# ZephirFXEC/HNanoSolver

Measured on AMD Instinct MI355X. Metric: solver substeps/sec (advect + 50 red-black SOR iterations + project) at N active voxels, higher is better.
Workload: dtype f32

## Files before the change

### hnanosolver_amd/_lib.py

```python
from __future__ import annotations

import ctypes as C
import os

_HERE = os.path.dirname(os.path.abspath(__file__))
_LIB_PATH = os.environ.get("HNS_LIBRARY") or os.path.join(_HERE, "lib", "libhns.so")

HNS_OK = 0
HNS_ERR_INVALID_ARGUMENT = -1
HNS_ERR_RUNTIME = -2
HNS_ERR_HIP = -3
HNS_ERR_NO_DEVICE = -4
HNS_ERR_TOPOLOGY = -5

HNS_GRID_DEFAULT = 0
HNS_GRID_HOST_ONLY = 1
HNS_GRID_SKIP_VALIDATE = 2


class HNSError(RuntimeError):

    def __init__(self, code: int, message: str):
        super().__init__(f"libhns error {code}: {message}")
        self.code = code
        self.message = message


class hns_field(C.Structure):
    _fields_ = [("name", C.c_char_p), ("ncomp", C.c_int), ("host", C.POINTER(C.c_float))]


class hns_dist_stats(C.Structure):
    _fields_ = [("world", C.c_int), ("rank", C.c_int), ("peers", C.c_int), ("sweeps_per_exchange", C.c_int),
                ("boundary_leaves", C.c_uint64), ("interior_leaves", C.c_uint64), ("ghost_leaves", C.c_uint64),
                ("region_voxels_sent", C.c_uint64 * 4), ("bytes_sent", C.c_uint64 * 4), ("messages_sent", C.c_uint64), ("exchanges", C.c_uint64),
                ("halo_peers", C.c_uint64), ("packed_exchanges", C.c_uint64), ("chained", C.c_uint64)]


HNS_DIST_IPC_BLOB_BYTES = 2048
HNS_DIST_PLAN_ONLY = 1
HNS_DIST_LEAF_ORDER = 2


class hns_leaf_source(C.Structure):
    _fields_ = [("name", C.c_char_p), ("ncomp", C.c_int), ("origins", C.c_void_p), ("n_leaves", C.c_uint64), ("masks", C.c_void_p), ("values", C.c_void_p)]


class hns_activity_field(C.Structure):
    _fields_ = [("name", C.c_char_p), ("ncomp", C.c_int), ("tolerance", C.c_float)]


class hns_combustion_params(C.Structure):
    _fields_ = [(n, C.c_float) for n in ("expansionRate", "temperatureRelease", "buoyancyStrength", "ambientTemp", "vorticityScale", "factorScale")]


_vp, _i, _u64, _f = C.c_void_p, C.c_int, C.c_uint64, C.c_float
_fp = C.c_void_p
_ip = C.POINTER(C.c_int)

SIGNATURES = {
    "hns_last_error": (C.c_char_p, []),
    "hns_version": (_i, []),
    "hns_device_count": (_i, []),
    "hns_trim_memory": (_i, []),
    "hns_set_option": (_i, [C.c_char_p, C.c_char_p]),
    "hns_get_option": (C.c_char_p, [C.c_char_p]),
    "hns_grid_create": (_vp, [_vp, _u64, _f, C.c_uint, _ip]),
    "hns_grid_create_from_leaves": (_vp, [_vp, _u64, _f, C.c_uint, _ip]),
    "hns_grid_destroy": (None, [_vp]),
    "hns_grid_leaf_count": (_u64, [_vp]),
    "hns_grid_voxel_count": (_u64, [_vp]),
    "hns_grid_voxel_size": (_f, [_vp]),
    "hns_grid_set_active_leaves": (_i, [_vp, _u64]),
    "hns_grid_set_active_range": (_i, [_vp, _u64, _u64]),
    "hns_grid_active_leaves": (_u64, [_vp]),
    "hns_grid_set_outside_element": (_i, [_vp, _u64]),
    "hns_grid_offsets": (_i, [_vp, _vp, _u64, _vp]),
    "hns_grid_neighbor_table": (_i, [_vp, _vp]),
    "hns_grid_coords": (_i, [_vp, _vp]),
    "hns_grid_release_cache": (_i, [_vp]),
    "hns_grid_matches": (_i, [_vp, _vp, _u64, C.c_uint]),
    "hns_grid_export_nanovdb": (_i, [_vp, _vp, _u64, _vp]),
    "hns_grid_launch_tables": (_i, [_vp, _vp]),
    "hns_gather_leaves": (_i, [_vp, _u64, _vp, _u64, _vp, _i, _i, _vp]),
    "hns_scatter_leaves": (_i, [_vp, _u64, _i, C.POINTER(C.c_void_p)]),
    "hns_dilate_leaves": (_i, [_vp, _u64, _vp, _i, _vp, _u64, C.POINTER(C.c_uint64)]),
    "hns_dilate_leaf_masks": (_i, [_vp, _u64, _vp, _i, _vp, _vp, _u64, C.POINTER(C.c_uint64)]),
    "hns_union_leaves": (_i, [_vp, _u64, _vp, _u64, _vp, _u64, C.POINTER(C.c_uint64)]),
    "hns_add_leaves": (_i, [_vp, _u64, _vp, _vp, _vp, _u64, _vp, _vp, _i, _vp, _vp, _vp, _u64, C.POINTER(C.c_uint64)]),
    "hns_deactivate_leaf_masks": (_i, [_u64, _vp, C.POINTER(hns_activity_field), C.POINTER(C.c_void_p), _i, _vp, C.POINTER(C.c_uint64)]),
    "hns_compute_sim": (_i, [_vp, C.POINTER(hns_field), _i, _i, _f, _f, C.POINTER(hns_combustion_params), _i, _vp]),
    "hns_compute_sim_resident": (_i, [_vp, C.POINTER(hns_field), _i, C.c_char_p, C.POINTER(C.c_int), _i, _f, _f, C.POINTER(hns_combustion_params), _i, _vp]),
    "hns_advect_index_grid": (_i, [_vp, C.POINTER(hns_field), _i, _f, _f, _vp]),
    "hns_advect_index_grid_velocity": (_i, [_vp, C.POINTER(hns_field), _i, _f, _f, _vp]),
    "hns_project_non_divergent": (_i, [_vp, C.POINTER(hns_field), _i, _u64, _f, _vp]),
    "hns_divergence": (_i, [_vp, C.POINTER(hns_field), _i, _f, _vp]),
    "hns_sim_create": (_vp, [_vp, C.POINTER(C.c_char_p), _i, _ip]),
    "hns_sim_destroy": (None, [_vp]),
    "hns_sim_upload": (_i, [_vp, C.POINTER(hns_field), _i, _vp]),
    "hns_sim_download": (_i, [_vp, C.POINTER(hns_field), _i, _vp]),
    "hns_sim_substep": (_i, [_vp, _i, _f, _f, C.POINTER(hns_combustion_params), _i, _vp]),
    "hns_sim_core_substep": (_i, [_vp, _i, _f, _f, _vp]),
    "hns_sim_pressure_solve": (_i, [_vp, _i, _f, _vp]),
    "hns_sim_timing": (_i, [_vp, _i]),
    "hns_sim_pressure_time": (_i, [_vp, C.POINTER(C.c_float), C.POINTER(C.c_longlong)]),
    "hns_sim_stage_timing": (_i, [_vp, _i]),
    "hns_sim_stage_times": (_i, [_vp, C.POINTER(C.c_float), C.POINTER(C.c_longlong)]),
    "hns_sim_velocity_ptr": (_vp, [_vp]),
    "hns_sim_field_ptr": (_vp, [_vp, C.c_char_p]),
    "hns_sim_divergence_ptr": (_vp, [_vp]),
    "hns_sim_pressure_ptr": (_vp, [_vp]),
    "hns_sim_set_active_masks": (_i, [_vp, _vp, _vp]),
    "hns_sim_active_masks": (_i, [_vp, _vp, _vp]),
    "hns_sim_regrid": (_vp, [_vp, _i, _vp, _u64, _vp, _vp, _vp, _ip]),
    "hns_sim_regrid_times": (_i, [_vp, C.POINTER(C.c_float)]),
    "hns_sim_regrid_sourced": (_vp, [_vp, _i, C.POINTER(hns_leaf_source), _i, _vp, _u64, _vp, _vp, _vp, _ip]),
    "hns_sim_deactivate": (_i, [_vp, C.POINTER(hns_activity_field), _i, C.POINTER(C.c_uint64), _vp]),
    "hns_dev_advect_vector": (_i, [_vp, _fp, _fp, _fp, _i, _f, _f, _vp]),
    "hns_dev_advect_scalar": (_i, [_vp, _fp, _fp, _fp, _fp, _i, _f, _f, _vp]),
    "hns_dev_advect_scalars": (_i, [_vp, _fp, C.POINTER(C.c_void_p), C.POINTER(C.c_void_p), _i, _fp, _i, _f, _f, _vp]),
    "hns_dev_divergence": (_i, [_vp, _fp, _fp, _f, _vp]),
    "hns_dev_rbgs_color": (_i, [_vp, _fp, _fp, _f, _f, _i, _vp]),
    "hns_dev_rbgs_iterate": (_i, [_vp, _fp, _fp, _fp, _f, _f, _i, _ip, _vp]),
    "hns_dev_subtract_pressure_gradient": (_i, [_vp, _fp, _fp, _fp, _fp, _i, _f, _vp]),
    "hns_dev_combustion_oxygen": (_i, [_fp] * 9 + [_f, _f, _u64, _vp]),
    "hns_dev_temperature_buoyancy": (_i, [_fp, _fp, _fp, _f, _f, _f, _u64, _vp]),
    "hns_dev_vorticity_confinement": (_i, [_vp, _fp, _fp, _f, _f, _f, _f, _vp]),
    "hns_dev_enforce_collision_boundaries": (_i, [_vp, _fp, _fp, _f, _vp]),
    "hns_dev_pack_leaves": (_i, [_fp, _vp, _u64, _fp, _i, _vp]),
    "hns_dev_unpack_leaves": (_i, [_fp, _vp, _u64, _fp, _i, _vp]),
    "hns_dist_create": (_vp, [_vp, _u64, _i, _i, _f, _i, _i, C.c_uint, _ip]),
    "hns_dist_destroy": (None, [_vp]),
    "hns_dist_unique_id": (_i, [_vp]),
    "hns_dist_connect_rccl": (_i, [_vp, _vp]),
    "hns_dist_connect_local": (_i, [C.POINTER(C.c_void_p), _i]),
    "hns_dist_connect_loopback": (_i, [_vp]),
    "hns_dist_connect_loopback_rccl": (_i, [_vp]),
    "hns_dist_ipc_export": (_i, [_vp, _vp]),
    "hns_dist_connect_ipc": (_i, [_vp, _vp]),
    "hns_dist_owned_leaves": (_u64, [_vp]),
    "hns_dist_first_owned_leaf": (_u64, [_vp]),
    "hns_dist_owned_leaf_ids": (_i, [_vp, _vp]),
    "hns_dist_partition_axis": (_i, [_vp]),
    "hns_dist_one_sided_sweeps": (_i, [_u64, _i]),
    "hns_dist_info": (_i, [_vp, C.POINTER(hns_dist_stats)]),
    "hns_dist_local_leaves": (_i, [_vp, _vp]),
    "hns_dist_peer_rank": (_i, [_vp, _i]),
    "hns_dist_peer_region": (_i, [_vp, _i, _i, _i, _vp, _vp, C.POINTER(C.c_uint64), C.POINTER(C.c_uint64)]),
    "hns_dist_upload": (_i, [_vp, _vp, C.POINTER(C.c_void_p), _vp]),
    "hns_dist_download": (_i, [_vp, _vp, C.POINTER(C.c_void_p), _vp, _vp]),
    "hns_dist_download_local": (_i, [_vp, _i, _vp, _vp]),
    "hns_dist_core_substep": (_i, [_vp, _i, _f, _vp]),
    "hns_dist_local_core_substep": (_i, [C.POINTER(C.c_void_p), _i, _i, _f, _vp]),
    "hns_dist_sim_substep": (_i, [_vp, _i, _f, _vp, _ip, _i, _vp]),
    "hns_dist_local_sim_substep": (_i, [C.POINTER(C.c_void_p), _i, _i, _f, _vp, _ip, _i, _vp]),
    "hns_dist_timing": (_i, [_vp, _i]),
    "hns_dist_pressure_time": (_i, [_vp, C.POINTER(C.c_float), C.POINTER(C.c_longlong)]),
    "hns_dist_synchronize": (_i, [_vp, _vp]),
    "hns_dev_time_rbgs": (_i, [_vp, _fp, _fp, _fp, _f, _f, _i, _i, C.POINTER(C.c_float), _vp]),
    "hns_grid_rbgs_plan": (_i, [_vp, _i, C.c_char_p, C.c_uint64, _ip, _ip]),
}

_lib = None


def library_path() -> str:
    return _LIB_PATH


def load_library() -> C.CDLL:
    global _lib
    if _lib is not None:
        return _lib
    if not os.path.exists(_LIB_PATH):
        raise FileNotFoundError(
            f"{_LIB_PATH} is missing: build it with `make -C hnanosolver_amd/csrc` (or `python -c 'import __graft_entry__ as g; g.build()'`). "
            "hnanosolver_amd has no CPU fallback."
        )
    lib_ = C.CDLL(_LIB_PATH, mode=C.RTLD_GLOBAL)
    for name, (res, args) in SIGNATURES.items():
        fn = getattr(lib_, name)
        fn.restype = res
        fn.argtypes = args
    _lib = lib_
    return lib_


class _LazyLib:
    def __getattr__(self, name):
        return getattr(load_library(), name)


lib = _LazyLib()


def set_option(name: str, value=None) -> None:
    check(load_library().hns_set_option(name.encode(), None if value is None else str(value).encode()))


def get_option(name: str):
    v = load_library().hns_get_option(name.encode())
    return None if v is None else v.decode()


def check(code: int) -> None:
    if code < 0:
        raise HNSError(code, load_library().hns_last_error().decode("utf-8", "replace"))
```

### hnanosolver_amd/csrc/hns_advect.hip

```cpp
#include <cstdlib>
#include <cstring>

#include "hns_device.hpp"

namespace hns {

struct Taps {
	int t[8];
	float fx, fy, fz;
};

typedef float v3f __attribute__((ext_vector_type(3)));
typedef int v4i __attribute__((ext_vector_type(4)));
__device__ v3f hns_buffer_load_v3f32(v4i rsrc, int voffset, int soffset, int aux) __asm("llvm.amdgcn.raw.buffer.load.v3f32");
__device__ float hns_buffer_load_f32(v4i rsrc, int voffset, int soffset, int aux) __asm("llvm.amdgcn.raw.buffer.load.f32");
typedef float v2f32 __attribute__((ext_vector_type(2)));
__device__ v2f32 hns_buffer_load_v2f32(v4i rsrc, int voffset, int soffset, int aux) __asm("llvm.amdgcn.raw.buffer.load.v2f32");
typedef float v4f32 __attribute__((ext_vector_type(4)));
__device__ v4f32 hns_buffer_load_v4f32(v4i rsrc, int voffset, int soffset, int aux) __asm("llvm.amdgcn.raw.buffer.load.v4f32");

constexpr unsigned kOutside = 0xFFFFE000u;
constexpr uint64_t kNarrowBytes = 0xFFFF0000ull;

__device__ __forceinline__ v4i field_rsrc(const float* p, unsigned bytes) {
// ... 223 lines not shown
}

constexpr int kBox = 1000, kBoxShell = kBox - 512;
constexpr int kVY = 24, kVX = 10 * kVY, kVP = 10 * kVX;
template <int XS = 100, int YS = 10>
__device__ __forceinline__ void box_shell_entry(int h, int& slot, int& local, int& cell) {
	int bx, by, bz;
	if (h < 200) {
		const int side = h >= 100, r = h - 100 * side;
		bx = 9 * side, by = r / 10, bz = r - 10 * by;
	} else if (h < 360) {
		const int q = h - 200, side = q >= 80, r = q - 80 * side;
		bx = 1 + r / 10, by = 9 * side, bz = r - 10 * (bx - 1);
	} else {
		const int q = h - 360, side = q >> 6, r = q & 63;
		bx = 1 + (r >> 3), by = 1 + (r & 7), bz = 9 * side;
	}
	slot = ((bx + 7) >> 3) * 9 + ((by + 7) >> 3) * 3 + ((bz + 7) >> 3);
	local = (((bx + 7) & 7) << 6) | (((by + 7) & 7) << 3) | ((bz + 7) & 7);
	cell = bx * XS + by * YS + bz;
}
__device__ __forceinline__ V3 box_v3(const float* s_box, int a) {
	V3 r;
	r.xy = v2f32{s_box[a], s_box[a + kVP]};
	r.z = s_box[a + 2 * kVP];
	return r;
}
__device__ __forceinline__ f3 tri_v_box(const float* s_box, int a, float fx, float fy, float fz) {
	V3 c[8];
#pragma unroll
	for (int q = 0; q < 8; ++q) c[q] = box_v3(s_box, a + (q >> 2) * kVX + ((q >> 1) & 1) * kVY + (q & 1));
	const V3 z0 = lerp_v3(c[0], c[1], fz), z1 = lerp_v3(c[2], c[3], fz), z2 = lerp_v3(c[4], c[5], fz), z3 = lerp_v3(c[6], c[7], fz);
	const V3 y0 = lerp_v3(z0, z1, fy), y1 = lerp_v3(z2, z3, fy);
	const V3 r = lerp_v3(y0, y1, fx);
	return f3{r.xy.x, r.xy.y, r.z};
}

__global__ __launch_bounds__(512) __attribute__((amdgpu_waves_per_eu(8, 8))) void k_advect_vector_n(const GridDev g, const float* __restrict__ u, float* __restrict__ out, const float scaled_dt) {
	__shared__ int s_nbr[27];
	__shared__ int s_base[27];
	__shared__ unsigned s_b4[27];
	__shared__ unsigned s_b4p[kPadTab];
	const int n = threadIdx.x;
	const int leaf = launch_leaf(g, blockIdx.x);
	const int idx = leaf * 512 + n;
	const v4i ru = field_rsrc(u, (unsigned)g.n_leaves * 6144u);
	const unsigned own = (unsigned)idx << 2;
	const f3 vo = ldv(ru, own);
	const LeafCtx L = stage_leaf_base(g, s_nbr, s_base, blockIdx.x, s_b4, s_b4p, leaf);
	const float px = (float)(L.org.x + (n >> 6)), py = (float)(L.org.y + ((n >> 3) & 7)), pz = (float)(L.org.z + (n & 7));

	__shared__ float s_box[3 * kVP];
	const int ob = ((n >> 6) + 1) * kVX + (((n >> 3) & 7) + 1) * kVY + (n & 7) + 1;
	s_box[ob] = vo.x, s_box[ob + kVP] = vo.y, s_box[ob + 2 * kVP] = vo.z;
	if (n < kBoxShell) {
		int slot, local, cell;
		box_shell_entry<kVX, kVY>(n, slot, local, cell);
		const f3 h = ldv(ru, s_b4[slot] + ((unsigned)local << 2));
		s_box[cell] = h.x, s_box[cell + kVP] = h.y, s_box[cell + 2 * kVP] = h.z;
	}
	float sx = px - scaled_dt * vo.x, sy = py - scaled_dt * vo.y, sz = pz - scaled_dt * vo.z;
	f3 vf = {0.0f, 0.0f, 0.0f}, vb = {0.0f, 0.0f, 0.0f};
	__syncthreads();
#pragma unroll 1
	for (int pass = 0; pass < 2; ++pass) {
		const int i = __float2int_rd(sx), j = __float2int_rd(sy), k = __float2int_rd(sz);
		const unsigned rx = (unsigned)(i - (L.org.x - 1)), ry = (unsigned)(j - (L.org.y - 1)), rz = (unsigned)(k - (L.org.z - 1));
		f3 v;
		if (__all(max(rx, max(ry, rz)) <= 8u)) {
			v = tri_v_box(s_box, (int)(rx * (unsigned)kVX + ry * (unsigned)kVY + rz), sx - (float)i, sy - (float)j, sz - (float)k);
		} else {
			const TapsB T = make_taps_b(g, s_nbr, s_b4p, L.org, sx, sy, sz);
			v = tri_v_b(ru, T);
		}
		if (pass == 0) {
			vf = v;
			sx = sx + scaled_dt * v.x, sy = sy + scaled_dt * v.y, sz = sz + scaled_dt * v.z;
		} else {
			vb = v;
		}
	}
	f3 vc = {vf.x + 0.5f * (vo.x - vb.x), vf.y + 0.5f * (vo.y - vb.y), vf.z + 0.5f * (vo.z - vb.z)};
	const int e[6] = {ob - kVX, ob + kVX, ob - kVY, ob + kVY, ob - 1, ob + 1};
	f3 mn = vo, mx = vo;
#pragma unroll
	for (int d = 0; d < 6; ++d) {
		const V3 t = box_v3(s_box, e[d]);
		mn.x = fminf(mn.x, t.xy.x);
		mx.x = fmaxf(mx.x, t.xy.x);
		mn.y = fminf(mn.y, t.xy.y);
		mx.y = fmaxf(mx.y, t.xy.y);
		mn.z = fminf(mn.z, t.z);
		mx.z = fmaxf(mx.z, t.z);
	}
	mn.x = fminf(mn.x, vf.x);
	mx.x = fmaxf(mx.x, vf.x);
	mn.y = fminf(mn.y, vf.y);
	mx.y = fmaxf(mx.y, vf.y);
	mn.z = fminf(mn.z, vf.z);
	mx.z = fmaxf(mx.z, vf.z);
	vc.x = fmaxf(mn.x, fminf(vc.x, mx.x));
	vc.y = fmaxf(mn.y, fminf(vc.y, mx.y));
	vc.z = fmaxf(mn.z, fminf(vc.z, mx.z));
	st3(out, idx, vc);
}

template <bool COLL>
__global__ __launch_bounds__(512) void k_advect_vector(const GridDev g, const float* __restrict__ u, float* __restrict__ out,
                                                       const float* __restrict__ sdf, const float scaled_dt, const float inv_dx) {
	__shared__ int s_nbr[27];
	__shared__ int s_base[27];
	const LeafCtx L = stage_leaf_base(g, s_nbr, s_base, blockIdx.x);
	const int n = threadIdx.x;
	const int idx = L.leaf * 512 + n;
	const int ci = L.org.x + (n >> 6), cj = L.org.y + ((n >> 3) & 7), ck = L.org.z + (n & 7);
	const float px = (float)ci, py = (float)cj, pz = (float)ck;

	const f3 vo = ld3(u, idx);
	float sx = px - scaled_dt * vo.x, sy = py - scaled_dt * vo.y, sz = pz - scaled_dt * vo.z;
	float rx = px, ry = py, rz = pz;
	f3 vf = {0.0f, 0.0f, 0.0f}, vb = {0.0f, 0.0f, 0.0f};
#pragma unroll 1
	for (int pass = 0; pass < 2; ++pass) {
		Taps T = make_taps(g, s_nbr, s_base, L.org, sx, sy, sz);
		if (COLL) {
			if (tri_f_t(sdf, T) < 0.0f) {
				sx = rx, sy = ry, sz = rz;
				T = make_taps(g, s_nbr, s_base, L.org, sx, sy, sz);
			}
		}
		const f3 v = tri_v_t(u, T);
		if (pass == 0) {
			vf = v;
			rx = sx, ry = sy, rz = sz;
			sx = sx + scaled_dt * v.x, sy = sy + scaled_dt * v.y, sz = sz + scaled_dt * v.z;
		} else {
			vb = v;
		}
	}
	f3 vc = {vf.x + 0.5f * (vo.x - vb.x), vf.y + 0.5f * (vo.y - vb.y), vf.z + 0.5f * (vo.z - vb.z)};

	int nb[6];
	nbr6(s_base, L.leaf, n, nb);
	f3 mn = vo, mx = vo;
#pragma unroll
	for (int d = 0; d < 6; ++d) {
		const f3 nv = ld3z(u, nb[d]);
		mn.x = fminf(mn.x, nv.x);
		mx.x = fmaxf(mx.x, nv.x);
		mn.y = fminf(mn.y, nv.y);
		mx.y = fmaxf(mx.y, nv.y);
		mn.z = fminf(mn.z, nv.z);
		mx.z = fmaxf(mx.z, nv.z);
	}
	mn.x = fminf(mn.x, vf.x);
	mx.x = fmaxf(mx.x, vf.x);
	mn.y = fminf(mn.y, vf.y);
	mx.y = fmaxf(mx.y, vf.y);
	mn.z = fminf(mn.z, vf.z);
	mx.z = fmaxf(mx.z, vf.z);
	vc.x = fmaxf(mn.x, fminf(vc.x, mx.x));
	vc.y = fmaxf(mn.y, fminf(vc.y, mx.y));
	vc.z = fmaxf(mn.z, fminf(vc.z, mx.z));

	if (COLL) {
		const float sv = sdf[idx];
		if (sv < 0.0f) {
			vc.x = vc.y = vc.z = 0.0f;
		} else if (sv < 0.1f) {
			const f3 nrm = sdf_normal(g, s_nbr, L.org, sdf, ci, cj, ck, inv_dx);
			vc = no_slip_blend(vc, nrm, 1.0f - (sv / 1.5f));
		}
	}
	st3(out, idx, vc);
}


__global__ __launch_bounds__(512) void k_advect_scalar_n(const GridDev g, const float* __restrict__ u, const float* __restrict__ in, float* __restrict__ out,
                                                         const float scaled_dt) {
	__shared__ int s_nbr[27];
	__shared__ int s_base[27];
	__shared__ unsigned s_b4[27];
	__shared__ unsigned s_b4p[kPadTab];
	const LeafCtx L = stage_leaf_base(g, s_nbr, s_base, blockIdx.x, s_b4, s_b4p);
	const int n = threadIdx.x;
	const int idx = L.leaf * 512 + n;
	const float px = (float)(L.org.x + (n >> 6)), py = (float)(L.org.y + ((n >> 3) & 7)), pz = (float)(L.org.z + (n & 7));
	const unsigned bytes1 = (unsigned)g.n_leaves * 2048u, own = (unsigned)idx << 2;
	const v4i ru = field_rsrc(u, bytes1 * 3u), rf = field_rsrc(in, bytes1);

	__shared__ float s_tile[kTile];
	const float phiOrig = lds1(rf, own);
	s_tile[n] = phiOrig;
	if (n < 384) s_tile[512 + n] = lds1(rf, halo_off(s_b4, n));
	const f3 vc = ldv(ru, own);
	float sx = px - scaled_dt * vc.x, sy = py - scaled_dt * vc.y, sz = pz - scaled_dt * vc.z;
	float phiForward = 0.0f, phiBackward = 0.0f;
#pragma unroll 1
	for (int pass = 0; pass < 2; ++pass) {
		const TapsB T = make_taps_b(g, s_nbr, s_b4p, L.org, sx, sy, sz);
		const float phi = tri_f_b(rf, T);
		if (pass == 0) {
			phiForward = phi;
			const f3 vf = tri_v_b(ru, T);
			sx = sx + scaled_dt * vf.x, sy = sy + scaled_dt * vf.y, sz = sz + scaled_dt * vf.z;
		} else {
			phiBackward = phi;
		}
	}
	const float error = phiOrig - phiBackward;
	const float phiCorr = phiForward + 0.5f * error;
	__syncthreads();
	const int e[6] = {tile_nbr<0, -1>(n), tile_nbr<0, 1>(n), tile_nbr<1, -1>(n), tile_nbr<1, 1>(n), tile_nbr<2, -1>(n), tile_nbr<2, 1>(n)};
	float mn = phiOrig, mx = phiOrig;
#pragma unroll
	for (int d = 0; d < 6; ++d) {
		const float nv = s_tile[e[d]];
		mn = fminf(mn, nv);
		mx = fmaxf(mx, nv);
	}
	mn = fminf(mn, phiForward);
	mx = fmaxf(mx, phiForward);
	out[idx] = fmaxf(mn, fminf(phiCorr, mx));
}

template <bool COLL>
__global__ __launch_bounds__(512) void k_advect_scalar(const GridDev g, const float* __restrict__ u, const float* __restrict__ in,
                                                       float* __restrict__ out, const float* __restrict__ sdf, const float scaled_dt) {
	__shared__ int s_nbr[27];
	__shared__ int s_base[27];
	const LeafCtx L = stage_leaf_base(g, s_nbr, s_base, blockIdx.x);
	const int n = threadIdx.x;
	const int idx = L.leaf * 512 + n;
	const int ci = L.org.x + (n >> 6), cj = L.org.y + ((n >> 3) & 7), ck = L.org.z + (n & 7);
	const float px = (float)ci, py = (float)cj, pz = (float)ck;

	const float phiOrig = in[idx];
	const f3 vc = ld3(u, idx);
	float sx = px - scaled_dt * vc.x, sy = py - scaled_dt * vc.y, sz = pz - scaled_dt * vc.z;
	float rx = px, ry = py, rz = pz;
	float phiForward = 0.0f, phiBackward = 0.0f;
#pragma unroll 1
	for (int pass = 0; pass < 2; ++pass) {
		Taps T = make_taps(g, s_nbr, s_base, L.org, sx, sy, sz);
		if (COLL) {
			if (tri_f_t(sdf, T) < 0.0f) {
				sx = rx, sy = ry, sz = rz;
				T = make_taps(g, s_nbr, s_base, L.org, sx, sy, sz);
			}
		}
		const float phi = tri_f_t(in, T);
		if (pass == 0) {
			phiForward = phi;
			const f3 vf = tri_v_t(u, T);
			rx = sx, ry = sy, rz = sz;
			sx = sx + scaled_dt * vf.x, sy = sy + scaled_dt * vf.y, sz = sz + scaled_dt * vf.z;
		} else {
			phiBackward = phi;
		}
	}
	const float error = phiOrig - phiBackward;
	const float phiCorr = phiForward + 0.5f * error;
	int nb[6];
	nbr6(s_base, L.leaf, n, nb);
	float mn = phiOrig, mx = phiOrig;
#pragma unroll
	for (int d = 0; d < 6; ++d) {
		const float nv = ldz(in, nb[d]);
		mn = fminf(mn, nv);
		mx = fmaxf(mx, nv);
	}
	mn = fminf(mn, phiForward);
	mx = fmaxf(mx, phiForward);
	out[idx] = fmaxf(mn, fminf(phiCorr, mx));
}


#define HNS_MAX_SCALARS 8
struct ScalarPtrs {
	const float* in[HNS_MAX_SCALARS];
	float* out[HNS_MAX_SCALARS];
	int n;
	const float* q4;
	float* q4_out[4];
};

__device__ __forceinline__ void interp_from_taps(const Taps& T, int oob, int (&ix)[8], float (&w)[8]) {
	const float tx = T.fx, ty = T.fy, tz = T.fz;
	const float itx = 1.0f - tx, ity = 1.0f - ty, itz = 1.0f - tz;
	const float w00 = itx * ity, w10 = tx * ity, w01 = itx * ty, w11 = tx * ty;
	w[0] = w00 * itz;
	w[1] = w10 * itz;
	w[2] = w01 * itz;
	w[3] = w11 * itz;
	w[4] = w00 * tz;
	w[5] = w10 * tz;
	w[6] = w01 * tz;
	w[7] = w11 * tz;
	const int perm[8] = {0, 4, 2, 6, 1, 5, 3, 7};
#pragma unroll
	for (int q = 0; q < 8; ++q) ix[q] = T.t[perm[q]] < 0 ? oob : T.t[perm[q]];
}

template <bool Q4>
__global__ __launch_bounds__(512) __attribute__((amdgpu_waves_per_eu(Q4 ? 6 : 4))) void k_advect_scalars_n(const GridDev g, const float* __restrict__ u, const ScalarPtrs P, const float scaled_dt) {
	__shared__ int s_nbr[27];
	__shared__ int s_base[27];
	__shared__ unsigned s_b4[27];
	__shared__ unsigned s_b4p[kPadTab];
	const int n = threadIdx.x;
	const int leaf = launch_leaf(g, blockIdx.x);
	const int idx = leaf * 512 + n;
	const unsigned bytes1 = (unsigned)g.n_leaves * 2048u;
	const v4i ru = field_rsrc(u, bytes1 * 3u);
	const unsigned own = (unsigned)idx << 2, oob4 = (unsigned)g.oob << 2;
	const f3 vc = ldv(ru, own);
	const LeafCtx L = stage_leaf_base(g, s_nbr, s_base, blockIdx.x, s_b4, s_b4p, leaf);
	const float px = (float)(L.org.x + (n >> 6)), py = (float)(L.org.y + ((n >> 3) & 7)), pz = (float)(L.org.z + (n & 7));

	const int ob = (((n >> 6) + 1) * 10 + ((n >> 3) & 7) + 1) * 10 + (n & 7) + 1;
	const int e[6] = {ob - 100, ob + 100, ob - 10, ob + 10, ob - 1, ob + 1};
	unsigned ho = 0u;
	int hcell = 0;
	if (n < kBoxShell) {
		int slot, local;
		box_shell_entry(n, slot, local, hcell);
		ho = s_b4[slot] + ((unsigned)local << 2);
	}
	ho = ho >= kOutside ? oob4 : ho;
	constexpr bool FIRST = Q4;
	__shared__ float s_ubox[FIRST ? 3 * kBox : 1];
	if constexpr (FIRST) {
		s_ubox[ob] = vc.x, s_ubox[ob + kBox] = vc.y, s_ubox[ob + 2 * kBox] = vc.z;
		if (n < kBoxShell) {
			const f3 h = ldv(ru, ho);
			s_ubox[hcell] = h.x, s_ubox[hcell + kBox] = h.y, s_ubox[hcell + 2 * kBox] = h.z;
		}
	}

	const float bx = px - scaled_dt * vc.x, by = py - scaled_dt * vc.y, bz = pz - scaled_dt * vc.z;
	unsigned bo[8], fo[8];
	float bw[8], fw[8];
	const int perm[8] = {0, 4, 2, 6, 1, 5, 3, 7};
	const int bi = __float2int_rd(bx), bj = __float2int_rd(by), bk = __float2int_rd(bz);
	const unsigned sx_ = (unsigned)(bi - (L.org.x - 1)), sy_ = (unsigned)(bj - (L.org.y - 1)), sz_ = (unsigned)(bk - (L.org.z - 1));
	const bool bboxed = FIRST && max(sx_, max(sy_, sz_)) <= 8u;
	const int ba = bboxed ? (int)((sx_ * 10u + sy_) * 10u + sz_) : 0;
	{
		float tx, ty, tz;
		if (bboxed) {
			tx = bx - (float)bi, ty = by - (float)bj, tz = bz - (float)bk;
#pragma unroll
			for (int q = 0; q < 8; ++q) bo[q] = 0u;
		} else {
			const TapsB T = make_taps_b(g, s_nbr, s_b4p, L.org, bx, by, bz);
			tx = T.fx, ty = T.fy, tz = T.fz;
#pragma unroll
			for (int q = 0; q < 8; ++q) bo[q] = T.o[perm[q]] >= kOutside ? oob4 : T.o[perm[q]];
		}
		const float itx = 1.0f - tx, ity = 1.0f - ty, itz = 1.0f - tz;
		const float w00 = itx * ity, w10 = tx * ity, w01 = itx * ty, w11 = tx * ty;
		bw[0] = w00 * itz, bw[1] = w10 * itz, bw[2] = w01 * itz, bw[3] = w11 * itz, bw[4] = w00 * tz, bw[5] = w10 * tz, bw[6] = w01 * tz, bw[7] = w11 * tz;
	}
	f3 vt[8];
	if (!bboxed) {
#pragma unroll
		for (int q = 0; q < 8; ++q) vt[q] = ldv(ru, bo[q]);
	}
	if constexpr (FIRST) __syncthreads();
	if (bboxed) {
#pragma unroll
		for (int q = 0; q < 8; ++q) {
			const int a = ba + (q & 1) * 100 + ((q >> 1) & 1) * 10 + (q >> 2);
			vt[q] = f3{s_ubox[a], s_ubox[a + kBox], s_ubox[a + 2 * kBox]};
		}
	}
	f3 vf = {0.0f, 0.0f, 0.0f};
#pragma unroll
	for (int q = 0; q < 8; ++q) {
		vf.x = vf.x + bw[q] * vt[q].x;
		vf.y = vf.y + bw[q] * vt[q].y;
		vf.z = vf.z + bw[q] * vt[q].z;
	}
	const float qx = bx + scaled_dt * vf.x, qy = by + scaled_dt * vf.y, qz = bz + scaled_dt * vf.z;
	const int qi = __float2int_rd(qx), qj = __float2int_rd(qy), qk = __float2int_rd(qz);
	const unsigned rx = (unsigned)(qi - (L.org.x - 1)), ry = (unsigned)(qj - (L.org.y - 1)), rz = (unsigned)(qk - (L.org.z - 1));
	const bool boxed = max(rx, max(ry, rz)) <= 8u;
	const int fa = boxed ? (int)((rx * 10u + ry) * 10u + rz) : 0;
	{
		float tx, ty, tz;
		if (boxed) {
			tx = qx - (float)qi, ty = qy - (float)qj, tz = qz - (float)qk;
#pragma unroll
			for (int q = 0; q < 8; ++q) fo[q] = 0u;
		} else {
			const TapsB T = make_taps_b(g, s_nbr, s_b4p, L.org, qx, qy, qz);
			tx = T.fx, ty = T.fy, tz = T.fz;
#pragma unroll
			for (int q = 0; q < 8; ++q) fo[q] = T.o[perm[q]] >= kOutside ? oob4 : T.o[perm[q]];
		}
		const float itx = 1.0f - tx, ity = 1.0f - ty, itz = 1.0f - tz;
		const float w00 = itx * ity, w10 = tx * ity, w01 = itx * ty, w11 = tx * ty;
		fw[0] = w00 * itz, fw[1] = w10 * itz, fw[2] = w01 * itz, fw[3] = w11 * itz, fw[4] = w00 * tz, fw[5] = w10 * tz, fw[6] = w01 * tz, fw[7] = w11 * tz;
	}
	__shared__ float s_box[2][kBox];
	if constexpr (Q4) {
		__shared__ v4f32 s_box4[kBox];
		const v4i rq = field_rsrc(P.q4, bytes1 * 4u);
		const v4f32 phiOrig = hns_buffer_load_v4f32(rq, (int)(own << 2), 0, 0);
		s_box4[ob] = phiOrig;
		if (n < kBoxShell) s_box4[hcell] = hns_buffer_load_v4f32(rq, (int)(ho << 2), 0, 0);
		v4f32 phiF = {0.0f, 0.0f, 0.0f, 0.0f}, phiB = {0.0f, 0.0f, 0.0f, 0.0f};
		if (!bboxed) {
			v4f32 c[8];
#pragma unroll
			for (int q = 0; q < 8; ++q) c[q] = hns_buffer_load_v4f32(rq, (int)(bo[q] << 2), 0, 0);
#pragma unroll
			for (int q = 0; q < 8; ++q) phiF = __builtin_elementwise_fma(c[q], v4f32{bw[q], bw[q], bw[q], bw[q]}, phiF);
		}
		if (!boxed) {
			v4f32 c[8];
#pragma unroll
			for (int q = 0; q < 8; ++q) c[q] = hns_buffer_load_v4f32(rq, (int)(fo[q] << 2), 0, 0);
#pragma unroll
			for (int q = 0; q < 8; ++q) phiB = __builtin_elementwise_fma(c[q], v4f32{fw[q], fw[q], fw[q], fw[q]}, phiB);
		}
		__syncthreads();
		if (bboxed) {
#pragma unroll
			for (int q = 0; q < 8; ++q) phiF = __builtin_elementwise_fma(s_box4[ba + (q & 1) * 100 + ((q >> 1) & 1) * 10 + (q >> 2)], v4f32{bw[q], bw[q], bw[q], bw[q]}, phiF);
		}
		if (boxed) {
#pragma unroll
			for (int q = 0; q < 8; ++q) phiB = __builtin_elementwise_fma(s_box4[fa + (q & 1) * 100 + ((q >> 1) & 1) * 10 + (q >> 2)], v4f32{fw[q], fw[q], fw[q], fw[q]}, phiB);
		}
		const v4f32 error = phiOrig - phiB;
		const v4f32 phiCorr = __builtin_elementwise_fma(v4f32{0.5f, 0.5f, 0.5f, 0.5f}, error, phiF);
		v4f32 mn = phiOrig, mx = phiOrig;
#pragma unroll
		for (int d = 0; d < 6; ++d) {
			const v4f32 v = s_box4[e[d]];
			mn = __builtin_elementwise_min(mn, v);
			mx = __builtin_elementwise_max(mx, v);
		}
		mn = __builtin_elementwise_min(mn, phiF);
		mx = __builtin_elementwise_max(mx, phiF);
		const v4f32 r = __builtin_elementwise_max(mn, __builtin_elementwise_min(phiCorr, mx));
		P.q4_out[0][idx] = r.x, P.q4_out[1][idx] = r.y, P.q4_out[2][idx] = r.z, P.q4_out[3][idx] = r.w;
	}
	for (int s = 0; s < P.n; ++s) {
		const v4i rf = field_rsrc(P.in[s], bytes1);
		float* box = s_box[s & 1];
		const float phiOrig = lds1(rf, own);
		box[ob] = phiOrig;
		if (n < kBoxShell) box[hcell] = lds1(rf, ho);
		float vb[8], vf8[8];
		if (!bboxed) {
#pragma unroll
			for (int q = 0; q < 4; ++q) ld_zpair(rf, bo[q], bo[q + 4], vb[q], vb[q + 4]);
		}
		if (!boxed) {
#pragma unroll
			for (int q = 0; q < 4; ++q) ld_zpair(rf, fo[q], fo[q + 4], vf8[q], vf8[q + 4]);
		}
		float phiF = 0.0f, phiB = 0.0f;
		__syncthreads();
		if (bboxed) {
#pragma unroll
			for (int q = 0; q < 8; ++q) vb[q] = box[ba + (q & 1) * 100 + ((q >> 1) & 1) * 10 + (q >> 2)];
		}
#pragma unroll
		for (int q = 0; q < 8; ++q) phiF = __fmaf_rn(vb[q], bw[q], phiF);
		if (boxed) {
#pragma unroll
			for (int q = 0; q < 8; ++q) vf8[q] = box[fa + (q & 1) * 100 + ((q >> 1) & 1) * 10 + (q >> 2)];
		}
#pragma unroll
		for (int q = 0; q < 8; ++q) phiB = __fmaf_rn(vf8[q], fw[q], phiB);
		const float error = phiOrig - phiB;
		const float phiCorr = __fmaf_rn(0.5f, error, phiF);
		float mn = phiOrig, mx = phiOrig;
#pragma unroll
		for (int d = 0; d < 6; ++d) {
			const float v = box[e[d]];
			mn = fminf(mn, v);
			mx = fmaxf(mx, v);
		}
		mn = fminf(mn, phiF);
		mx = fmaxf(mx, phiF);
		P.out[s][idx] = fmaxf(mn, fminf(phiCorr, mx));
	}
}

template <bool COLL>
__global__ __launch_bounds__(512) void k_advect_scalars(const GridDev g, const float* __restrict__ u, const ScalarPtrs P,
                                                        const float* __restrict__ sdf, const float scaled_dt) {
	__shared__ int s_nbr[27];
	__shared__ int s_base[27];
	const LeafCtx L = stage_leaf_base(g, s_nbr, s_base, blockIdx.x);
	const int n = threadIdx.x;
	const int idx = L.leaf * 512 + n;
	const int ci = L.org.x + (n >> 6), cj = L.org.y + ((n >> 3) & 7), ck = L.org.z + (n & 7);
	const float px = (float)ci, py = (float)cj, pz = (float)ck;

	const f3 vc = ld3(u, idx);
	float sx = px - scaled_dt * vc.x, sy = py - scaled_dt * vc.y, sz = pz - scaled_dt * vc.z;
	float rx = px, ry = py, rz = pz;
	int bi[8], fi[8];
	float bw[8], fw[8];
#pragma unroll 1
	for (int pass = 0; pass < 2; ++pass) {
		Taps T = make_taps(g, s_nbr, s_base, L.org, sx, sy, sz);
		if (COLL) {
			if (tri_f_t(sdf, T) < 0.0f) {
				sx = rx, sy = ry, sz = rz;
				T = make_taps(g, s_nbr, s_base, L.org, sx, sy, sz);
			}
		}
		if (pass == 0) {
			interp_from_taps(T, g.oob, bi, bw);
			f3 vf = {0.0f, 0.0f, 0.0f};
#pragma unroll
			for (int q = 0; q < 8; ++q) {
				const f3 v = ld3(u, bi[q]);
				vf.x = vf.x + bw[q] * v.x;
				vf.y = vf.y + bw[q] * v.y;
				vf.z = vf.z + bw[q] * v.z;
			}
			rx = sx, ry = sy, rz = sz;
			sx = sx + scaled_dt * vf.x, sy = sy + scaled_dt * vf.y, sz = sz + scaled_dt * vf.z;
		} else {
			interp_from_taps(T, g.oob, fi, fw);
		}
	}
	int nb[6];
	nbr6(s_base, L.leaf, n, nb);
#pragma unroll
	for (int d = 0; d < 6; ++d) nb[d] = nb[d] < 0 ? g.oob : nb[d];
	for (int s = 0; s < P.n; ++s) {
		const float* __restrict__ in = P.in[s];
		const float phiOrig = in[idx];
		float phiF = 0.0f, phiB = 0.0f;
#pragma unroll
		for (int q = 0; q < 8; ++q) {
			phiF = __fmaf_rn(in[bi[q]], bw[q], phiF);
			phiB = __fmaf_rn(in[fi[q]], fw[q], phiB);
		}
		const float error = phiOrig - phiB;
		const float phiCorr = __fmaf_rn(0.5f, error, phiF);
		float mn = phiOrig, mx = phiOrig;
#pragma unroll
		for (int d = 0; d < 6; ++d) {
			const float v = in[nb[d]];
			mn = fminf(mn, v);
			mx = fmaxf(mx, v);
		}
		mn = fminf(mn, phiF);
		mx = fmaxf(mx, phiF);
		P.out[s][idx] = fmaxf(mn, fminf(phiCorr, mx));
	}
}

}

using namespace hns;

static bool narrow_fields(const hns_grid* g) {
	return !options().advect_generic.load() && (uint64_t)g->topo.n_leaves * 6144u <= hns::kNarrowBytes;
}

extern "C" {

int hns_dev_advect_vector(hns_grid* g, const float* vel3, float* out3, const float* sdf, int has_collision, float dt, float inv_dx, void* stream) {
	if (int rc = check_grid(g, "hns_dev_advect_vector")) return rc;
	NULLCHK(!vel3 || !out3, "hns_dev_advect_vector");
	if (vel3 == out3) return fail(HNS_ERR_INVALID_ARGUMENT, "hns_dev_advect_vector: output must not alias input");
	if (g->n_active == 0) return HNS_OK;
	const float scaled_dt = dt * inv_dx;
	const dim3 grid((unsigned)g->n_active), block(512);
	if (has_collision && sdf)
		hipLaunchKernelGGL(k_advect_vector<true>, grid, block, 0, (hipStream_t)stream, g->dev(), vel3, out3, sdf, scaled_dt, inv_dx);
	else if (narrow_fields(g))
		hipLaunchKernelGGL(k_advect_vector_n, grid, block, 0, (hipStream_t)stream, g->dev(), vel3, out3, scaled_dt);
	else
		hipLaunchKernelGGL(k_advect_vector<false>, grid, block, 0, (hipStream_t)stream, g->dev(), vel3, out3, sdf, scaled_dt, inv_dx);
	return launch_status("hns_dev_advect_vector");
}

int hns_dev_advect_scalar(hns_grid* g, const float* vel3, const float* in, float* out, const float* sdf, int has_collision, float dt, float inv_dx,
                          void* stream) {
	if (int rc = check_grid(g, "hns_dev_advect_scalar")) return rc;
	NULLCHK(!vel3 || !in || !out, "hns_dev_advect_scalar");
	if (g->n_active == 0) return HNS_OK;
	const float scaled_dt = dt * inv_dx;
	const dim3 grid((unsigned)g->n_active), block(512);
	if (has_collision && sdf)
		hipLaunchKernelGGL(k_advect_scalar<true>, grid, block, 0, (hipStream_t)stream, g->dev(), vel3, in, out, sdf, scaled_dt);
	else if (narrow_fields(g))
		hipLaunchKernelGGL(k_advect_scalar_n, grid, block, 0, (hipStream_t)stream, g->dev(), vel3, in, out, scaled_dt);
	else
		hipLaunchKernelGGL(k_advect_scalar<false>, grid, block, 0, (hipStream_t)stream, g->dev(), vel3, in, out, sdf, scaled_dt);
	return launch_status("hns_dev_advect_scalar");
}

int hns_dev_advect_scalars(hns_grid* g, const float* vel3, const float* const* in, float* const* out, int n, const float* sdf, int has_collision,
                           float dt, float inv_dx, void* stream) {
	if (int rc = check_grid(g, "hns_dev_advect_scalars")) return rc;
	NULLCHK(!vel3 || (n > 0 && (!in || !out)), "hns_dev_advect_scalars");
	if (g->n_active == 0 || n <= 0) return HNS_OK;
	const float scaled_dt = dt * inv_dx;
	const dim3 grid((unsigned)g->n_active), block(512);
	for (int base = 0; base < n; base += HNS_MAX_SCALARS) {
		ScalarPtrs P;
		P.n = n - base < HNS_MAX_SCALARS ? n - base : HNS_MAX_SCALARS;
		for (int s = 0; s < HNS_MAX_SCALARS; ++s) {
			P.q4 = nullptr, P.q4_out[0] = P.q4_out[1] = P.q4_out[2] = P.q4_out[3] = nullptr;
			P.in[s] = s < P.n ? in[base + s] : nullptr;
			P.out[s] = s < P.n ? out[base + s] : nullptr;
			if (s < P.n && (!P.in[s] || !P.out[s])) {
				set_error("hns_dev_advect_scalars: null device pointer for field %d", base + s);
				return HNS_ERR_INVALID_ARGUMENT;
			}
		}
		if (has_collision && sdf)
			hipLaunchKernelGGL(k_advect_scalars<true>, grid, block, 0, (hipStream_t)stream, g->dev(), vel3, P, sdf, scaled_dt);
		else if (narrow_fields(g))
		{
			GridDev gd = g->dev();
			gd.rev = 1;
			hipLaunchKernelGGL(k_advect_scalars_n<false>, grid, block, 0, (hipStream_t)stream, gd, vel3, P, scaled_dt);
		}
		else
			hipLaunchKernelGGL(k_advect_scalars<false>, grid, block, 0, (hipStream_t)stream, g->dev(), vel3, P, sdf, scaled_dt);
	}
	return launch_status("hns_dev_advect_scalars");
}

int hns_advect_scalars_q4(hns_grid* g, const float* vel3, const float* q4, float* const* q4_out, const float* const* in, float* const* out, int n, float dt, float inv_dx,
                          void* stream) {
	if (int rc = check_grid(g, "hns_advect_scalars_q4")) return rc;
	NULLCHK(!vel3 || !q4 || !q4_out || (n > 0 && (!in || !out)), "hns_advect_scalars_q4");
	if (!hns_advect_q4_ok(g) || n > HNS_MAX_SCALARS) return fail(HNS_ERR_INVALID_ARGUMENT, "hns_advect_scalars_q4: grid too large for 32-bit offsets, or too many fields");
	if (g->n_active == 0) return HNS_OK;
	ScalarPtrs P;
	P.n = n;
	P.q4 = q4;
	for (int c = 0; c < 4; ++c) {
		NULLCHK(!q4_out[c], "hns_advect_scalars_q4");
		P.q4_out[c] = q4_out[c];
	}
	for (int s = 0; s < HNS_MAX_SCALARS; ++s) {
		P.in[s] = s < n ? in[s] : nullptr;
		P.out[s] = s < n ? out[s] : nullptr;
		NULLCHK(s < n && (!P.in[s] || !P.out[s]), "hns_advect_scalars_q4");
	}
	GridDev gd = g->dev();
	gd.rev = 1;
	hipLaunchKernelGGL(k_advect_scalars_n<true>, dim3((unsigned)g->n_active), dim3(512), 0, (hipStream_t)stream, gd, vel3, P, dt * inv_dx);
	return launch_status("hns_advect_scalars_q4");
}

bool hns_advect_q4_ok(const hns_grid* g) { return narrow_fields(g) && (uint64_t)g->topo.n_leaves * 8192u <= hns::kNarrowBytes; }

}
```

### hnanosolver_amd/csrc/hns_api.hip

```cpp
#include <algorithm>
#include <cstdlib>
#include <cstring>
#include <string>
#include <thread>
#include <vector>

#include "hns_internal.hpp"
#include "hns_digest.hpp"

using namespace hns;


GridDev hns_grid::dev() const {
	GridDev d;
	d.origins = (const int4*)d_origins;
	d.nbr27 = (const int*)d_nbr27;
	d.hash = (const int*)d_hash;
	d.sched = (const int*)d_sched;
	d.sched_seg = sched_seg, d.sched_pre = sched_pre;
	d.blk = (const int*)d_blk;
	d.hash_mask = topo.hash_mask;
	d.n_leaves = (int)topo.n_leaves;
	d.n_active = (int)n_active;
	d.first = (int)first_active;
	d.oob = (int)outside_element;
	d.rev = 0;
	d.far_flag = far_flag;
	return d;
}

extern "C" int hns_device_count(void) {
	int n = 0;
	if (hipGetDeviceCount(&n) != hipSuccess) return 0;
	return n;
}



extern "C" void hns_sim_destroy(hns_sim* s) {
	if (!s) return;
	s->solve_ev.destroy();
	s->stage_ev.destroy();
	for (hipEvent_t e : s->xev)
		if (e) (void)hipEventDestroy(e);
	for (hipEvent_t e : s->rev)
		if (e) (void)hipEventDestroy(e);
	if (s->xfer) (void)hipStreamDestroy(s->xfer);
	if (s->h_dig) (void)hipHostFree(s->h_dig);
	hns_arena_put(s->d_masks, s->masks_bytes, s->device);
	hns_arena_put(s->d_act, s->act_bytes, s->device);
	hns_arena_put(s->arena, s->arena_bytes, s->device);
	delete s;
}

extern "C" int hns_grid_release_cache(hns_grid* g) {
	if (!g) return fail(HNS_ERR_INVALID_ARGUMENT, "hns_grid_release_cache: null grid");
	std::vector<hns_sim*> drop;
	{
		std::lock_guard<std::mutex> lock(g->host_mutex);
		for (size_t i = 0; i < g->sim_cache.size();) {
			if (g->sim_cache[i]->in_use) {
				++i;
				continue;
			}
			drop.push_back(g->sim_cache[i]);
			g->sim_cache.erase(g->sim_cache.begin() + (long)i);
		}
	}
	for (hns_sim* s : drop) {
		s->cached = false;
		hns_sim_destroy(s);
	}
	return HNS_OK;
}

static size_t sim_unit(uint64_t n) { return (sizeof(float) * (size_t)(n ? n : 1) + 255) & ~(size_t)255; }
static bool sim_combust(const hns_sim* s) { return std::all_of(kCombustionFields, kCombustionFields + 4, [s](const char* n) { return s->find(n) >= 0; }); }
static size_t sim_units(const hns_sim* s) { return 3 * 3 + 3 + 2 * s->names.size() + (sim_combust(s) ? 4 : 0); }

size_t hns_sim_arena_need(const hns_sim* s, uint64_t n) { return sim_unit(n) * sim_units(s) + 256; }

void hns_sim_layout(hns_sim* s, void* arena, uint64_t n) {
	const size_t unit = sim_unit(n);
	char* q = (char*)arena;
	auto take = [&](size_t k) {
		float* r = (float*)q;
		q += k * unit;
		return r;
	};
	s->n = n;
	s->vel = take(3), s->adv = take(3), s->tmp = take(3);
	s->div = take(1), s->p_a = take(1), s->p_b = take(1);
	s->cur.clear(), s->nxt.clear();
	for (size_t i = 0; i < s->names.size(); ++i) {
		s->cur.push_back(take(1));
		s->nxt.push_back(take(1));
	}
	s->q4 = sim_combust(s) ? take(4) : nullptr;
	s->d_dig = (unsigned long long*)q;
	s->p_result = s->p_a;
}

static hns_sim* sim_create(hns_grid* g, const char* const* float_names, int n_float, bool zero, void* stream, int* rc_out) {
	hns_sim* s = new hns_sim;
	s->grid = g;
	s->n = hns_grid_voxel_count(g);
	s->device = g->device;
	int rc = HNS_OK;
	for (int i = 0; i < n_float && rc == HNS_OK; ++i) {
		if (!float_names[i]) {
			rc = fail(HNS_ERR_INVALID_ARGUMENT, "hns_sim_create: null field name");
		} else if (s->find(float_names[i]) >= 0) {
			set_error("hns_sim_create: duplicate field name '%s'", float_names[i]);
			rc = HNS_ERR_INVALID_ARGUMENT;
		} else {
			s->names.push_back(float_names[i]);
		}
	}
	s->handed_cur.resize(s->names.size());
	void* arena = nullptr;
	size_t bytes = 0;
	if (rc == HNS_OK) rc = hns_arena_get(hns_sim_arena_need(s, s->n), s->device, &arena, &bytes);
	if (rc == HNS_OK) {
		s->arena = arena, s->arena_bytes = bytes;
		hns_sim_layout(s, s->arena, s->n);
		if (zero && hipMemsetAsync(s->arena, 0, (char*)s->d_dig - (char*)s->arena, (hipStream_t)stream) != hipSuccess) rc = fail(HNS_ERR_HIP, "hns_sim_create: clearing the field memory failed");
	}
	if (rc != HNS_OK) {
		hns_sim_destroy(s);
		s = nullptr;
	}
	*rc_out = rc;
	return s;
}

extern "C" hns_sim* hns_sim_create(hns_grid* g, const char* const* float_names, int n_float, int* err) {
	int rc = HNS_OK;
	if (!g || n_float < 0 || (n_float > 0 && !float_names)) {
		rc = fail(HNS_ERR_INVALID_ARGUMENT, "hns_sim_create: bad arguments");
	} else if (!g->on_device) {
		rc = fail(HNS_ERR_NO_DEVICE, "hns_sim_create: grid has no device tables (there is no CPU fallback)");
	}
	if (rc != HNS_OK) {
		if (err) *err = rc;
		return nullptr;
	}
	hns_sim* s = sim_create(g, float_names, n_float, true, nullptr, &rc);
	if (s && hipStreamSynchronize(nullptr) != hipSuccess) {
		rc = fail(HNS_ERR_HIP, "hns_sim_create: clearing the field memory failed");
		hns_sim_destroy(s);
		s = nullptr;
	}
	if (err) *err = rc;
	return s;
}

static int sim_field(hns_sim* s, const hns_field& f, const char* who, int* k, float** buf) {
	if (f.ncomp == 3) {
		*k = hns_sim::kVelocity, *buf = s->vel;
		return HNS_OK;
	}
	if (f.ncomp != 1) {
		set_error("%s: ncomp must be 1 or 3", who);
		return HNS_ERR_INVALID_ARGUMENT;
	}
	*k = f.name ? s->find(f.name) : -1;
	if (*k < 0) {
		set_error("%s: no float field named '%s' in this sim", who, f.name ? f.name : "?");
		return HNS_ERR_RUNTIME;
	}
	*buf = s->cur[*k];
	return HNS_OK;
}

extern "C" int hns_sim_upload(hns_sim* s, const hns_field* fields, int n_fields, void* stream) {
	if (!s || (n_fields > 0 && !fields)) return fail(HNS_ERR_INVALID_ARGUMENT, "hns_sim_upload: null argument");
	for (int i = 0; i < n_fields; ++i) {
		const hns_field& f = fields[i];
		if (!f.host) {
			set_error("hns_sim_upload: host pointer is null for block: %s", f.name ? f.name : "?");
			return HNS_ERR_RUNTIME;
		}
		int k;
		float* buf;
		HNS_TRY(sim_field(s, f, "hns_sim_upload", &k, &buf));
		s->forget(k);
		HNS_HIP(hipMemcpyAsync(buf, f.host, sizeof(float) * (size_t)f.ncomp * (size_t)s->n, hipMemcpyHostToDevice, (hipStream_t)stream));
	}
	return HNS_OK;
}

extern "C" int hns_sim_download(hns_sim* s, hns_field* fields, int n_fields, void* stream) {
	if (!s || (n_fields > 0 && !fields)) return fail(HNS_ERR_INVALID_ARGUMENT, "hns_sim_download: null argument");
	for (int i = 0; i < n_fields; ++i) {
		hns_field& f = fields[i];
		if (!f.host) return fail(HNS_ERR_RUNTIME, "hns_sim_download: null host pointer");
		int k;
		float* buf;
		HNS_TRY(sim_field(s, f, "hns_sim_download", &k, &buf));
		HNS_HIP(hipMemcpyAsync(f.host, buf, sizeof(float) * (size_t)f.ncomp * (size_t)s->n, hipMemcpyDeviceToHost, (hipStream_t)stream));
	}
	HNS_HIP(hipStreamSynchronize((hipStream_t)stream));
	return HNS_OK;
}

extern "C" float* hns_sim_velocity_ptr(hns_sim* s) { return s ? s->vel : nullptr; }
extern "C" float* hns_sim_field_ptr(hns_sim* s, const char* name) {
	if (!s || !name) return nullptr;
	const int k = s->find(name);
	return k < 0 ? nullptr : s->cur[k];
}
extern "C" float* hns_sim_divergence_ptr(hns_sim* s) { return s ? s->div : nullptr; }
extern "C" float* hns_sim_pressure_ptr(hns_sim* s) { return s ? s->p_result : nullptr; }

static int validate_step(float voxel_size, float dt, int64_t iterations, bool need_iter) {
	if (voxel_size <= 0.0f) return fail(HNS_ERR_INVALID_ARGUMENT, "voxelSize must be positive.");
	if (dt < 0.0f) return fail(HNS_ERR_INVALID_ARGUMENT, "dt (time step) cannot be negative.");
	if (need_iter && iterations <= 0) return fail(HNS_ERR_INVALID_ARGUMENT, "Number of pressure iterations must be positive.");
	return HNS_OK;
}

static int sim_pressure(hns_sim* s, int iterations, float voxel_size, float omega, void* stream) {
	int in_b = 0;
	hipEvent_t* timed = s->solve_ev.current();
	if (timed) HNS_HIP(hipEventRecord(timed[0], (hipStream_t)stream));
	HNS_TRY(hns_rbgs_iterate(s->grid, s->div, s->p_a, s->p_b, voxel_size, omega, iterations, &in_b, stream, true));
	if (timed) {
		HNS_HIP(hipEventRecord(timed[1], (hipStream_t)stream));
		s->solve_ev.advance();
		s->timed_launches += iterations;
	}
	s->p_result = in_b ? s->p_b : s->p_a;
	return HNS_OK;
}

namespace hns {
float omega_compute(float vs) { return 2.0f / (1.0f + sinf(static_cast<float>(3.14159) * vs)); }
}
static float omega_project(float vs) { return (float)(2.0f / (1.0f + sin(3.14159 * (double)vs))); }

extern "C" int hns_sim_pressure_solve(hns_sim* s, int iterations, float voxel_size, void* stream) {
	if (!s) return fail(HNS_ERR_INVALID_ARGUMENT, "hns_sim_pressure_solve: null sim");
	HNS_TRY(validate_step(voxel_size, 0.0f, iterations, true));
	return sim_pressure(s, iterations, voxel_size, omega_compute(voxel_size), stream);
}

extern "C" int hns_sim_timing(hns_sim* s, int max_solves) {
	if (!s || max_solves < 0) return fail(HNS_ERR_INVALID_ARGUMENT, "hns_sim_timing: bad arguments");
	s->timed_launches = 0;
	return s->solve_ev.reset(max_solves);
}

extern "C" int hns_sim_stage_timing(hns_sim* s, int max_substeps) {
	if (!s || max_substeps < 0) return fail(HNS_ERR_INVALID_ARGUMENT, "hns_sim_stage_timing: bad arguments");
	return s->stage_ev.reset(max_substeps);
}

extern "C" int hns_sim_stage_times(hns_sim* s, float* ms5, long long* substeps) {
	if (!s || !ms5 || !substeps) return fail(HNS_ERR_INVALID_ARGUMENT, "hns_sim_stage_times: null argument");
	double tot[5];
	HNS_TRY(s->stage_ev.elapsed(tot));
	for (int k = 0; k < 5; ++k) ms5[k] = (float)tot[k];
	*substeps = (long long)s->stage_ev.used;
	return HNS_OK;
}

extern "C" int hns_sim_pressure_time(hns_sim* s, float* total_ms, long long* launches) {
	if (!s || !total_ms || !launches) return fail(HNS_ERR_INVALID_ARGUMENT, "hns_sim_pressure_time: null argument");
	double tot;
	HNS_TRY(s->solve_ev.elapsed(&tot));
	*total_ms = (float)tot;
	*launches = s->timed_launches;
	return HNS_OK;
}

static int sim_advect_scalars(hns_sim* s, const float* sdf, bool coll, float dt, float inv_dx, void* stream) {
	std::vector<const float*> ins;
	std::vector<float*> outs;
	std::vector<int> which;
	for (size_t i = 0; i < s->names.size(); ++i) {
		if (s->names[i] == "collision_sdf") continue;
		ins.push_back(s->cur[i]);
		outs.push_back(s->nxt[i]);
		which.push_back((int)i);
	}
	HNS_TRY(hns_dev_advect_scalars(s->grid, s->vel, ins.data(), outs.data(), (int)ins.size(), sdf, coll, dt, inv_dx,
	                               stream));
	for (int i : which) std::swap(s->cur[i], s->nxt[i]);
	return HNS_OK;
}

namespace {
struct Substep {
	hns_sim* s;
	int iterations;
	float dt, voxel_size, inv_dx;
	const hns_combustion_params* params;
	int ci[4];
	bool coll = false, fused = false;
	const float* sdf = nullptr;
	void* stream;
	hipEvent_t* stage_events = nullptr;
	bool full() const { return params != nullptr; }
	int mark(int k) {
		if (stage_events) HNS_HIP(hipEventRecord(stage_events[k], (hipStream_t)stream));
		return HNS_OK;
	}

	int prepare(hns_sim* sim, int iters, float dt_, float vs, const hns_combustion_params* prm, int has_collision, void* st) {
		s = sim;
		iterations = iters;
		dt = dt_;
		voxel_size = vs;
		inv_dx = 1.0f / vs;
		params = prm;
		stream = st;
		if (!full()) return HNS_OK;
		if (s->names.empty()) return fail(HNS_ERR_RUNTIME, "No float blocks found in input data.");
		for (int c = 0; c < 4; ++c) {
			ci[c] = s->find(kCombustionFields[c]);
			if (ci[c] < 0) {
				set_error("Missing required input field for combustion: %s", kCombustionFields[c]);
				return HNS_ERR_RUNTIME;
			}
		}
		const int i_sdf = has_collision ? s->find("collision_sdf") : -1;
		coll = i_sdf >= 0;
		sdf = coll ? s->cur[i_sdf] : nullptr;
		size_t advected = 0;
		for (const std::string& n : s->names) advected += n != "collision_sdf";
		fused = !coll && s->q4 && s->grid->d_blk && s->grid->n_active == (uint64_t)s->grid->topo.n_leaves && !options().stencil_block.load() && hns_advect_q4_ok(s->grid) &&
		        advected - 4 <= 8 && options().fuse_pointwise.load();
		return HNS_OK;
	}
	int part_a() {
		hns_grid* g = s->grid;
		HNS_TRY(mark(0));
		if (coll) HNS_TRY(hns_dev_enforce_collision_boundaries(g, s->vel, sdf, voxel_size, stream));
		HNS_TRY(hns_dev_advect_vector(g, s->vel, s->adv, sdf, coll, dt, inv_dx, stream));
		if (full() && (int)params->factorScale != 0) {
			HNS_TRY(hns_dev_vorticity_confinement(g, s->adv, s->tmp, dt, inv_dx,
			                                      params->vorticityScale, params->factorScale, stream));
			std::swap(s->adv, s->tmp);
		}
		return HNS_OK;
	}
	int part_b() {
		hns_grid* g = s->grid;
		HNS_TRY(mark(1));
		if (fused) {
			HNS_TRY(hns_divergence_combust_buoyancy(g, s->adv, s->div, inv_dx, s->cur[ci[0]], s->cur[ci[1]], s->cur[ci[2]], s->cur[ci[3]], s->q4, s->tmp,
			                                        params->temperatureRelease, params->expansionRate, dt, params->ambientTemp, params->buoyancyStrength, stream));
			std::swap(s->adv, s->tmp);
		} else {
			HNS_TRY(hns_dev_divergence(g, s->adv, s->div, inv_dx, stream));
			if (full()) {
				HNS_TRY(hns_dev_combustion_oxygen(s->cur[ci[0]], s->cur[ci[1]], s->cur[ci[2]], s->div, s->cur[ci[3]], s->nxt[ci[0]], s->nxt[ci[1]],
				                                  s->nxt[ci[2]], s->nxt[ci[3]], params->temperatureRelease, params->expansionRate, s->n, stream));
				HNS_TRY(hns_dev_temperature_buoyancy(s->adv, s->nxt[ci[2]], s->adv, dt, params->ambientTemp, params->buoyancyStrength, s->n,
				                                     stream));
				for (int c = 0; c < 4; ++c) std::swap(s->cur[ci[c]], s->nxt[ci[c]]);
			}
		}
		HNS_TRY(mark(2));
		HNS_TRY(sim_pressure(s, iterations, voxel_size, omega_compute(voxel_size), stream));
		HNS_TRY(mark(3));
		HNS_TRY(hns_dev_subtract_pressure_gradient(g, s->adv, s->p_result, s->vel, sdf, coll,
		                                           inv_dx, stream));
		if (coll) HNS_TRY(hns_dev_enforce_collision_boundaries(g, s->vel, sdf, voxel_size, stream));
		return HNS_OK;
	}
	int part_c() {
		HNS_TRY(mark(4));
		if (!fused) return sim_advect_scalars(s, sdf, coll, dt, inv_dx, stream);
		std::vector<const float*> ins;
		std::vector<float*> outs;
		float* q4_out[4];
		for (int c = 0; c < 4; ++c) q4_out[c] = s->nxt[ci[c]];
		for (size_t i = 0; i < s->names.size(); ++i) {
			if (s->names[i] == "collision_sdf" || (int)i == ci[0] || (int)i == ci[1] || (int)i == ci[2] || (int)i == ci[3]) continue;
			ins.push_back(s->cur[i]);
			outs.push_back(s->nxt[i]);
		}
		HNS_TRY(hns_advect_scalars_q4(s->grid, s->vel, s->q4, q4_out, ins.data(), outs.data(), (int)ins.size(), dt, inv_dx, stream));
		for (size_t i = 0; i < s->names.size(); ++i)
			if (s->names[i] != "collision_sdf") std::swap(s->cur[i], s->nxt[i]);
		return HNS_OK;
	}
	int run() {
		stage_events = s->stage_ev.current();
		HNS_TRY(part_a());
		HNS_TRY(part_b());
		HNS_TRY(part_c());
		HNS_TRY(mark(5));
		if (stage_events) s->stage_ev.advance();
		return HNS_OK;
	}
};

int sim_substep(hns_sim* s, int iterations, float dt, float voxel_size, const hns_combustion_params* params, int has_collision, void* stream) {
	HNS_TRY(validate_step(voxel_size, dt, iterations, true));
	if (s->n == 0) return HNS_OK;
	Substep step;
	HNS_TRY(step.prepare(s, iterations, dt, voxel_size, params, has_collision, stream));
	return step.run();
}
}

extern "C" int hns_sim_substep(hns_sim* s, int iterations, float dt, float voxel_size, const hns_combustion_params* params, int has_collision,
                               void* stream) {
	if (!s || !params) return fail(HNS_ERR_INVALID_ARGUMENT, "hns_sim_substep: null argument");
	return sim_substep(s, iterations, dt, voxel_size, params, has_collision, stream);
}

extern "C" int hns_sim_core_substep(hns_sim* s, int iterations, float dt, float voxel_size, void* stream) {
	if (!s) return fail(HNS_ERR_INVALID_ARGUMENT, "hns_sim_core_substep: null sim");
	return sim_substep(s, iterations, dt, voxel_size, nullptr, 0, stream);
}


namespace {
struct FieldSplit {
	hns_field* velocity = nullptr;
	int n_vec3 = 0;
	std::vector<hns_field*> floats;
};

int split_fields(hns_field* fields, int n_fields, FieldSplit& out, const char* who) {
	if (n_fields < 0 || (n_fields > 0 && !fields)) {
		set_error("%s: null field array", who);
		return HNS_ERR_INVALID_ARGUMENT;
	}
	for (int i = 0; i < n_fields; ++i) {
		if (fields[i].ncomp == 3) {
			if (!out.velocity) out.velocity = &fields[i];
			++out.n_vec3;
		} else if (fields[i].ncomp == 1) {
			out.floats.push_back(&fields[i]);
		} else {
			set_error("%s: field %d has ncomp %d (must be 1 or 3)", who, i, fields[i].ncomp);
			return HNS_ERR_INVALID_ARGUMENT;
		}
		if (!fields[i].name) {
			set_error("%s: field %d has no name", who, i);
			return HNS_ERR_INVALID_ARGUMENT;
		}
	}
	return HNS_OK;
}

struct SimGuard {
	hns_sim* s = nullptr;
	~SimGuard() {
		if (!s) return;
		if (!s->cached) {
			hns_sim_destroy(s);
			return;
		}
		std::lock_guard<std::mutex> lock(s->grid->host_mutex);
		s->in_use = false;
	}
};

int make_sim(hns_grid* g, const std::vector<hns_field*>& floats, SimGuard& guard, void* stream) {
	std::vector<const char*> names;
	for (hns_field* f : floats) names.push_back(f->name);
	const bool use_cache = options().cook_cache.load() != 0;
	if (use_cache) {
		std::lock_guard<std::mutex> lock(g->host_mutex);
		for (hns_sim* c : g->sim_cache) {
			if (c->in_use || c->names.size() != names.size()) continue;
			bool same = true;
			for (size_t i = 0; i < names.size() && same; ++i) same = c->names[i] == names[i];
			if (!same) continue;
			c->in_use = true;
			guard.s = c;
			break;
		}
	}
	if (guard.s) {
		if (g->n_active != (uint64_t)g->topo.n_leaves) {
			hns_sim* s = guard.s;
			const size_t bytes = sizeof(float) * (size_t)s->n;
			hipStream_t st = (hipStream_t)stream;
			HNS_HIP(hipMemsetAsync(s->div, 0, bytes, st));
			HNS_HIP(hipMemsetAsync(s->p_a, 0, bytes, st));
			HNS_HIP(hipMemsetAsync(s->p_b, 0, bytes, st));
			HNS_HIP(hipMemsetAsync(s->adv, 0, 3 * bytes, st));
			HNS_HIP(hipMemsetAsync(s->tmp, 0, 3 * bytes, st));
			for (float* q : s->nxt) HNS_HIP(hipMemsetAsync(q, 0, bytes, st));
		}
		return HNS_OK;
	}
	int err = HNS_OK;
	guard.s = sim_create(g, names.data(), (int)names.size(), g->n_active != (uint64_t)g->topo.n_leaves, stream, &err);
	if (err != HNS_OK || !use_cache) return err;
	std::lock_guard<std::mutex> lock(g->host_mutex);
	if (g->sim_cache.size() >= 2) {
		for (size_t i = 0; i < g->sim_cache.size(); ++i)
			if (!g->sim_cache[i]->in_use) {
				g->sim_cache[i]->cached = false;
				hns_sim_destroy(g->sim_cache[i]);
				g->sim_cache.erase(g->sim_cache.begin() + (long)i);
				break;
			}
	}
	if (g->sim_cache.size() < 2) {
		guard.s->cached = guard.s->in_use = true;
		g->sim_cache.push_back(guard.s);
	}
	return HNS_OK;
}

int operator_fields(hns_grid* g, hns_field* fields, int n_fields, const char* who, FieldSplit& fs) {
	if (!g) {
		set_error("%s: null grid", who);
		return HNS_ERR_INVALID_ARGUMENT;
	}
	HNS_TRY(split_fields(fields, n_fields, fs, who));
	if (fs.n_vec3 != 1) return fail(HNS_ERR_RUNTIME, "Expected exactly one Vec3f block (velocity)");
	return HNS_OK;
}

int operator_sim(hns_grid* g, const char* who, const std::vector<hns_field*>& floats, const hns_field* up, int n_up, SimGuard& guard, void* stream) {
	if (hns_grid_voxel_count(g) == 0) return HNS_OK;
	if (!g->on_device) {
		set_error("%s: grid has no device tables (there is no CPU fallback)", who);
		return HNS_ERR_NO_DEVICE;
	}
	HNS_TRY(make_sim(g, floats, guard, stream));
	return hns_sim_upload(guard.s, up, n_up, stream);
}
}

static uint64_t host_signature(const float* a, size_t count) {
	uint64_t h = 1469598103934665603ull ^ (uint64_t)count;
	const size_t samples = count < 4096 ? count : 4096;
	for (size_t i = 0; i < samples; ++i) {
		uint32_t bits;
		memcpy(&bits, a + (samples == count ? i : (size_t)(((unsigned __int128)i * count) / samples)), 4);
		h = (h ^ bits) * 1099511628211ull;
	}
	return h ? h : 1;
}
static uint64_t host_digest(const float* a, size_t count) {
	const size_t n_pieces = count / 4;
	constexpr size_t kChunk = (size_t)1 << 14;
	const size_t n_chunks = (n_pieces + kChunk - 1) / kChunk;
	std::vector<uint64_t> part(std::max<size_t>(1, n_chunks), 0);
	auto work = [&](size_t c0, size_t c1) {
		for (size_t c = c0; c < c1; ++c) {
			const size_t lo = c * kChunk, hi = std::min(n_pieces, lo + kChunk);
			uint64_t s0 = 0, s1 = 0;
			size_t i = lo;
			for (; i + 2 <= hi; i += 2) {
				uint64_t w[4];
				memcpy(w, a + 4 * i, 32);
				s0 += hns_digest_piece(i, w[0], w[1]);
				s1 += hns_digest_piece(i + 1, w[2], w[3]);
			}
			for (; i < hi; ++i) {
				uint64_t w[2];
				memcpy(w, a + 4 * i, 16);
				s0 += hns_digest_piece(i, w[0], w[1]);
			}
			part[c] = s0 + s1;
		}
	};
	const size_t n_threads = std::min<size_t>(8, std::max<size_t>(1, n_chunks / 8));
	if (n_threads <= 1) work(0, n_chunks);
	else {
		std::vector<std::thread> th;
		for (size_t t = 1; t < n_threads; ++t) th.emplace_back(work, n_chunks * t / n_threads, n_chunks * (t + 1) / n_threads);
		work(0, n_chunks / n_threads);
		for (auto& t : th) t.join();
	}
	uint64_t sum = 0;
	for (uint64_t p : part) sum += p;
	if (count & 3) {
		uint32_t w[4] = {0, 0, 0, 0};
		memcpy(w, a + 4 * n_pieces, 4 * (count & 3));
		sum += hns_digest_piece(n_pieces, (uint64_t)w[0] | (uint64_t)w[1] << 32, (uint64_t)w[2] | (uint64_t)w[3] << 32);
	}
	return hns_digest_finish(sum, count);
}

namespace {
struct Cook {
	hns_sim* s;
	const hns_field* fields;
	int n_fields;
	FieldSplit& fs;
	const unsigned char* resident;
	int* skipped;
	int iterations;
	float dt, voxel_size;
	const hns_combustion_params* params;
	int has_collision;
	hipStream_t st;
	std::vector<std::pair<uint64_t*, size_t>> dig_slots = {};

	size_t count() const { return (size_t)s->n; }
	int level_of(const hns_field* f) const { return resident ? resident[f - fields] : 0; }
	static bool is_sdf(const hns_field* f) { return !strcmp(f->name, "collision_sdf"); }
	static bool is_combustion_field(const hns_field* f) {
		return std::any_of(kCombustionFields, kCombustionFields + 4, [f](const char* n) { return !strcmp(f->name, n); });
	}

	bool stays(const hns_field* f) {
		const int level = level_of(f);
		if (!level) return false;
		hns_sim::Handed have;
		const size_t n = (size_t)f->ncomp * count();
		if (f->ncomp == 3) have = s->handed_vel;
		else if (const int k = s->find(f->name); k >= 0) have = s->handed_cur[(size_t)k];
		if (!have.sig || have.sig != host_signature(f->host, n)) return false;
		if (level >= 2 && (!have.dig || have.dig != host_digest(f->host, n))) return false;
		if (skipped) ++*skipped;
		return true;
	}
	int upload(hns_field* f, hipStream_t on) { return stays(f) ? (int)HNS_OK : hns_sim_upload(s, f, 1, on); }

	int digest_on_device(hipStream_t on) {
		std::vector<const float*> bufs;
		if (level_of(fs.velocity) >= 2) bufs.push_back(s->vel), dig_slots.emplace_back(&s->handed_vel.dig, 3 * count());
		for (hns_field* f : fs.floats) {
			const int k = s->find(f->name);
			if (k >= 0 && !is_sdf(f) && level_of(f) >= 2) bufs.push_back(s->cur[(size_t)k]), dig_slots.emplace_back(&s->handed_cur[(size_t)k].dig, count());
		}
		if (bufs.empty()) return HNS_OK;
		if (!s->h_dig) HNS_HIP(hipHostMalloc((void**)&s->h_dig, sizeof(unsigned long long) * 16, hipHostMallocDefault));
		HNS_HIP(hipMemsetAsync(s->d_dig, 0, sizeof(unsigned long long) * 16, on));
		for (size_t i = 0; i < bufs.size(); ++i) HNS_TRY(hns_field_digest(bufs[i], dig_slots[i].second, s->d_dig + i, on));
		HNS_HIP(hipMemcpyAsync(s->h_dig, s->d_dig, sizeof(unsigned long long) * 16, hipMemcpyDeviceToHost, on));
		return HNS_OK;
	}
	int sign() {
		s->handed_vel = {host_signature(fs.velocity->host, 3 * count()), 0};
		for (hns_field* f : fs.floats) {
			const int k = s->find(f->name);
			if (k >= 0) s->handed_cur[(size_t)k] = {is_sdf(f) ? 0 : host_signature(f->host, count()), 0};
		}
		for (size_t i = 0; i < dig_slots.size(); ++i) *dig_slots[i].first = hns_digest_finish(s->h_dig[i], dig_slots[i].second);
		return HNS_OK;
	}

	int plain() {
		std::vector<hns_field> all;
		HNS_TRY(upload(fs.velocity, st));
		all.push_back(*fs.velocity);
		for (hns_field* f : fs.floats) {
			HNS_TRY(upload(f, st));
			all.push_back(*f);
		}
		HNS_TRY(hns_sim_substep(s, iterations, dt, voxel_size, params, has_collision, st));
		HNS_TRY(digest_on_device(st));
		HNS_TRY(hns_sim_download(s, all.data(), (int)all.size(), st));
		return sign();
	}

	static int handoff(hipEvent_t e, hipStream_t from, hipStream_t to) {
		HNS_HIP(hipEventRecord(e, from));
		HNS_HIP(hipStreamWaitEvent(to, e, 0));
		return HNS_OK;
	}
	int pipelined() {
		if (!s->xfer) {
			HNS_HIP(hipStreamCreateWithFlags(&s->xfer, hipStreamNonBlocking));
			for (hipEvent_t& e : s->xev) HNS_HIP(hipEventCreateWithFlags(&e, hipEventDisableTiming));
		}
		hipStream_t xf = s->xfer;
		Substep step;
		HNS_TRY(step.prepare(s, iterations, dt, voxel_size, params, has_collision, st));
		HNS_TRY(handoff(s->xev[0], st, xf));
		if (step.coll)
			for (hns_field* f : fs.floats)
				if (is_sdf(f)) HNS_TRY(hns_sim_upload(s, f, 1, xf));
		HNS_TRY(upload(fs.velocity, xf));
		HNS_TRY(handoff(s->xev[1], xf, st));
		HNS_TRY(step.part_a());
		for (hns_field* f : fs.floats)
			if (is_combustion_field(f)) HNS_TRY(upload(f, xf));
		HNS_TRY(handoff(s->xev[2], xf, st));
		HNS_TRY(step.part_b());
		HNS_HIP(hipEventRecord(s->xev[3], st));
		for (hns_field* f : fs.floats)
			if (!is_combustion_field(f) && !is_sdf(f)) HNS_TRY(upload(f, xf));
		HNS_TRY(handoff(s->xev[4], xf, st));
		HNS_TRY(step.part_c());
		HNS_TRY(digest_on_device(st));
		HNS_HIP(hipStreamWaitEvent(xf, s->xev[3], 0));
		HNS_HIP(hipMemcpyAsync(fs.velocity->host, s->vel, sizeof(float) * 3 * count(), hipMemcpyDeviceToHost, xf));
		HNS_TRY(handoff(s->xev[0], st, xf));
		std::vector<hns_field> outs;
		for (hns_field* f : fs.floats)
			if (!is_sdf(f)) outs.push_back(*f);
		HNS_TRY(hns_sim_download(s, outs.data(), (int)outs.size(), xf));
		HNS_HIP(hipStreamSynchronize(st));
		return sign();
	}

	int run() {
		int checked = 0;
		for (int i = 0; resident && i < n_fields; ++i) checked += resident[i] >= 2 ? 1 : 0;
		if (checked > 16) return fail(HNS_ERR_INVALID_ARGUMENT, "hns_compute_sim_resident: more than 16 CHECKED fields");
		return options().cook_pipeline.load() ? pipelined() : plain();
	}
};
}

extern "C" int hns_compute_sim(hns_grid* g, hns_field* fields, int n_fields, int iterations, float dt, float voxel_size,
                               const hns_combustion_params* params, int has_collision, void* stream) {
	return hns_compute_sim_resident(g, fields, n_fields, nullptr, nullptr, iterations, dt, voxel_size, params, has_collision, stream);
}

extern "C" int hns_compute_sim_resident(hns_grid* g, hns_field* fields, int n_fields, const unsigned char* resident, int* uploads_skipped, int iterations, float dt,
                                        float voxel_size, const hns_combustion_params* params, int has_collision, void* stream) {
	if (uploads_skipped) *uploads_skipped = 0;
	HNS_TRY(validate_step(voxel_size, dt, iterations, true));
	if (!g) return fail(HNS_ERR_INVALID_ARGUMENT, "Invalid grid handle provided (null grid).");
	if (!params) return fail(HNS_ERR_INVALID_ARGUMENT, "hns_compute_sim: null combustion params");
	if (hns_grid_voxel_count(g) == 0) return HNS_OK;
	FieldSplit fs;
	HNS_TRY(split_fields(fields, n_fields, fs, "hns_compute_sim"));
	if (fs.n_vec3 != 1) {
		set_error("Expected exactly one Vec3f block (velocity), found %d", fs.n_vec3);
		return HNS_ERR_RUNTIME;
	}
	if (!fs.velocity->host) return fail(HNS_ERR_RUNTIME, "Host velocity data pointer is null");
	if (fs.floats.empty()) return fail(HNS_ERR_RUNTIME, "No float blocks found in input data.");
	for (hns_field* f : fs.floats)
		if (!f->host) {
			set_error("Host float data pointer is null for block: %s", f->name);
			return HNS_ERR_RUNTIME;
		}
	if (!g->on_device) return fail(HNS_ERR_NO_DEVICE, "hns_compute_sim: grid has no device tables (there is no CPU fallback)");
	SimGuard guard;
	HNS_TRY(make_sim(g, fs.floats, guard, stream));
	Cook cook{guard.s, fields, n_fields, fs, resident, uploads_skipped, iterations, dt, voxel_size, params, has_collision, (hipStream_t)stream};
	if (int rc = cook.run()) {
		guard.s->forget();
		if (guard.s->xfer) (void)hipStreamSynchronize(guard.s->xfer);
		(void)hipStreamSynchronize((hipStream_t)stream);
		return rc;
	}
	for (hns_field* f : fs.floats)
		if (strcmp(f->name, "collision_sdf") == 0) memset(f->host, 0, sizeof(float) * (size_t)hns_grid_voxel_count(g));
	return HNS_OK;
}

extern "C" int hns_advect_index_grid(hns_grid* g, hns_field* fields, int n_fields, float dt, float voxel_size, void* stream) {
	FieldSplit fs;
	HNS_TRY(operator_fields(g, fields, n_fields, "hns_advect_index_grid", fs));
	if (fs.floats.empty()) return fail(HNS_ERR_RUNTIME, "No float blocks found");
	if (!fs.velocity->host) return fail(HNS_ERR_RUNTIME, "Velocity data not found");
	for (hns_field* f : fs.floats)
		if (!f->host) {
			set_error("Block '%s' not found or type mismatch", f->name);
			return HNS_ERR_RUNTIME;
		}
	SimGuard guard;
	HNS_TRY(operator_sim(g, "hns_advect_index_grid", fs.floats, fields, n_fields, guard, stream));
	hns_sim* s = guard.s;
	if (!s) return HNS_OK;
	const float inv_dx = 1.0f / voxel_size;
	for (size_t i = 0; i < s->names.size(); ++i) {
		HNS_TRY(hns_dev_advect_scalar(g, s->vel, s->cur[i], s->nxt[i], nullptr, 0, dt, inv_dx, stream));
		std::swap(s->cur[i], s->nxt[i]);
	}
	std::vector<hns_field> outs;
	for (hns_field* f : fs.floats) outs.push_back(*f);
	return hns_sim_download(s, outs.data(), (int)outs.size(), stream);
}

extern "C" int hns_advect_index_grid_velocity(hns_grid* g, hns_field* fields, int n_fields, float dt, float voxel_size, void* stream) {
	FieldSplit fs;
	HNS_TRY(operator_fields(g, fields, n_fields, "hns_advect_index_grid_velocity", fs));
	if (!fs.velocity->host) return fail(HNS_ERR_RUNTIME, "Velocity data not found");
	SimGuard guard;
	HNS_TRY(operator_sim(g, "hns_advect_index_grid_velocity", {}, fs.velocity, 1, guard, stream));
	hns_sim* s = guard.s;
	if (!s) return HNS_OK;
	HNS_TRY(hns_dev_advect_vector(g, s->vel, s->adv, nullptr, 0, dt, 1.0f / voxel_size, stream));
	std::swap(s->vel, s->adv);
	return hns_sim_download(s, fs.velocity, 1, stream);
}

extern "C" int hns_project_non_divergent(hns_grid* g, hns_field* fields, int n_fields, uint64_t iterations, float voxel_size, void* stream) {
	FieldSplit fs;
	HNS_TRY(operator_fields(g, fields, n_fields, "hns_project_non_divergent", fs));
	if (!fs.velocity->host) return fail(HNS_ERR_RUNTIME, "Velocity data not found");
	if (voxel_size <= 0.0f) return fail(HNS_ERR_INVALID_ARGUMENT, "voxelSize must be positive.");
	if (iterations > 0x7fffffffull) return fail(HNS_ERR_INVALID_ARGUMENT, "hns_project_non_divergent: iteration count too large");
	SimGuard guard;
	HNS_TRY(operator_sim(g, "hns_project_non_divergent", {}, fs.velocity, 1, guard, stream));
	hns_sim* s = guard.s;
	if (!s) return HNS_OK;
	const float inv_dx = 1.0f / voxel_size;
// ... 26 lines not shown
```

### hnanosolver_amd/csrc/hns_internal.hpp

```cpp
#pragma once

#include <hip/hip_runtime.h>

#include <algorithm>
#include <atomic>
#include <cstdarg>
#include <cstdint>
#include <cstdio>
#include <mutex>
#include <string>
#include <vector>

#include "hns.h"

namespace hns {

void set_error(const char* fmt, ...);
inline int fail(int code, const char* msg) {
	set_error("%s", msg);
	return code;
}

#define HNS_TRY(call)                    \
	do {                                 \
		int rc__ = (call);               \
		if (rc__ != HNS_OK) return rc__; \
	} while (0)

#define HNS_HIP(call)                                                                                   \
	do {                                                                                                \
		hipError_t e__ = (call);                                                                        \
		if (e__ != hipSuccess) {                                                                        \
			hns::set_error("%s failed: %s (%s:%d)", #call, hipGetErrorString(e__), __FILE__, __LINE__); \
			return HNS_ERR_HIP;                                                                         \
		}                                                                                               \
	} while (0)

constexpr const char* kCombustionFields[4] = {"fuel", "waste", "temperature", "flame"};

struct EventGroups {
	size_t per;
	std::vector<hipEvent_t> ev;
	size_t used = 0;
	bool on = false;
	explicit EventGroups(size_t per_) : per(per_) {}
	int reset(int groups) {
		while (ev.size() < (size_t)groups * per) {
			hipEvent_t e;
			HNS_HIP(hipEventCreate(&e));
			ev.push_back(e);
		}
		on = groups > 0;
		used = 0;
		return HNS_OK;
	}
	hipEvent_t* current() { return on && (used + 1) * per <= ev.size() ? &ev[used * per] : nullptr; }
	void advance() { ++used; }
	int elapsed(double* ms) {
		std::fill(ms, ms + per - 1, 0.0);
		for (size_t g = 0; g < used; ++g) {
			const hipEvent_t* e = &ev[g * per];
			HNS_HIP(hipEventSynchronize(e[per - 1]));
			for (size_t k = 0; k + 1 < per; ++k) {
				float t = 0.0f;
				HNS_HIP(hipEventElapsedTime(&t, e[k], e[k + 1]));
				ms[k] += t;
			}
		}
		return HNS_OK;
	}
	void destroy() {
		for (hipEvent_t e : ev) (void)hipEventDestroy(e);
		ev.clear();
	}
};

struct DeviceScope {
	int prev = -1;
	bool switched = false;
	explicit DeviceScope(int device) {
		if (device >= 0 && hipGetDevice(&prev) == hipSuccess && prev != device) switched = hipSetDevice(device) == hipSuccess;
	}
	~DeviceScope() {
		if (switched) (void)hipSetDevice(prev);
	}
};

enum { kRbgsAuto = 0, kRbgsColor = 1 };
enum { kScheduleAuto = 0, kScheduleLinear = 1 };
struct Options {
	std::atomic<int> rbgs{kRbgsAuto};
	std::atomic<int> advect_generic{0};
	std::atomic<int> stencil_block{0};
	std::atomic<int> schedule{kScheduleAuto};
	std::atomic<int> cook_cache{1};
	std::atomic<int> cook_pipeline{1};
	std::atomic<int> divergence_form{0};
	std::atomic<int> fuse_pointwise{1};
	std::atomic<int> sor_block_lb{0};
	std::atomic<int> dist_wire_us{0};
	std::atomic<int> dist_mirror{1};
	std::atomic<int> dist_unsplit{1};
};
Options& options();

struct Topology {
	std::vector<int32_t> origins;
	std::vector<int32_t> nbr27;
	std::vector<int32_t> hash;
	uint32_t hash_mask = 0;
	int64_t n_leaves = 0;
	bool have_tables = false;

	int prepare(const int32_t* leaf_origins_xyz, int64_t n_leaves);
	int build_tables();
	int64_t find_leaf(int32_t ox, int32_t oy, int32_t oz) const;
	uint64_t offset(int32_t i, int32_t j, int32_t k) const;
};

uint32_t hash_origin(int32_t x, int32_t y, int32_t z);
void sort_leaf_origins(int32_t* xyz, size_t n);

struct GridDev {
	const int4* origins;
	const int* nbr27;
	const int* hash;
	const int* sched;
	int sched_seg;
	int sched_pre;
	const int* blk;
	uint32_t hash_mask;
	int n_leaves;
	int n_active;
	int first;
	int oob;
	int rev;
	int* far_flag;
};

__device__ __forceinline__ unsigned launch_pos(const GridDev& g, unsigned b) {
	if (!g.rev) return b;
	const unsigned rows = (unsigned)g.n_active >> 3;
	return (b >> 3) < rows ? (((rows - 1u - (b >> 3)) << 3) | (b & 7u)) : b;
}

__device__ __forceinline__ int launch_leaf(const GridDev& g, unsigned b) {
	const int pos = (int)launch_pos(g, b);
	if (g.sched_seg == 0 && g.sched_pre == 0) {
		const int base = g.n_active >> 3, rem = g.n_active & 7, x = pos & 7, i = pos >> 3;
		return g.first + x * base + (x < rem ? x : rem) + i;
	}
	return g.sched ? g.sched[pos] : g.first + pos;
}

}

struct hns_sim;

struct hns_grid {
	hns::Topology topo;
	float voxel_size = 1.0f;
	uint64_t n_active = 0;
	uint64_t first_active = 0;
	uint64_t outside_element = 0;
	int* far_flag = nullptr;
	bool on_device = false;
	int device = -1;
	void* d_origins = nullptr;
	void* d_nbr27 = nullptr;
	void* d_hash = nullptr;
	void* d_sched = nullptr;
	void* d_blk = nullptr;
	int sched_seg = -1, sched_pre = 0;
	uint64_t chain_boundary = 0;
	uint64_t sched_prefix = 0;
	void* d_sched_mem = nullptr;
	void* d_scratch = nullptr;
	void* d_arena = nullptr;
	size_t arena_bytes = 0;
	void* d_sb_tab = nullptr;
	size_t sb_bytes = 0;
	uint64_t n_sb = 0;
	bool sb_built = false;
	int sb_seg = 0;
	uint64_t sb_first = 0, sb_count = 0;
	std::vector<std::pair<void*, size_t>> sb_retired;
	std::mutex build_mutex;
	std::mutex host_mutex;
	std::vector<hns_sim*> sim_cache;
	hns::GridDev dev() const;
};

struct hns_sim {
	hns_grid* grid = nullptr;
	uint64_t n = 0;
	std::vector<std::string> names;
	std::vector<float*> cur;
	std::vector<float*> nxt;
	float* vel = nullptr;
	float* adv = nullptr;
	float* tmp = nullptr;
	float* q4 = nullptr;
	float* div = nullptr;
	float* p_a = nullptr;
	float* p_b = nullptr;
	float* p_result = nullptr;
	hns::EventGroups solve_ev{2};
	long long timed_launches = 0;
	hns::EventGroups stage_ev{6};
	hipStream_t xfer = nullptr;
	hipEvent_t xev[5] = {nullptr, nullptr, nullptr, nullptr, nullptr};
	bool cached = false, in_use = false;
	struct Handed { uint64_t sig = 0, dig = 0; };
	Handed handed_vel;
	std::vector<Handed> handed_cur;
	static constexpr int kVelocity = -1, kEverything = -2;
	void forget(int k = kEverything) {
		if (k == kEverything || k == kVelocity) handed_vel = Handed{};
		for (size_t i = 0; i < handed_cur.size(); ++i)
			if (k == kEverything || k == (int)i) handed_cur[i] = Handed{};
	}
	unsigned long long* d_dig = nullptr;
	unsigned long long* h_dig = nullptr;
	void* arena = nullptr;
	size_t arena_bytes = 0;
	unsigned char* d_masks = nullptr;
	size_t masks_bytes = 0;
	hipEvent_t rev[6] = {nullptr, nullptr, nullptr, nullptr, nullptr, nullptr};
	bool regrid_timed = false;
	void* d_act = nullptr;
	size_t act_bytes = 0;
	int device = -1;
	int find(const char* name) const {
		for (size_t i = 0; i < names.size(); ++i)
			if (names[i] == name) return (int)i;
		return -1;
	}
};

namespace hns { int check_activity_fields(const hns_sim* s, const hns_activity_field* fields, int n_fields, const char* who, std::vector<int>* field_of); }

size_t hns_sim_arena_need(const hns_sim* s, uint64_t n);
void hns_sim_layout(hns_sim* s, void* arena, uint64_t n);

extern "C" __attribute__((visibility("hidden"))) int hns_rbgs_iterate(hns_grid* g, const float* div, float* p_a, float* p_b, float dx, float omega, int iterations, int* result_in_b,
                                void* stream, bool from_zero);

namespace hns { struct PhaseMirror; struct PackMirror; }
extern "C" __attribute__((visibility("hidden"))) int hns_rbgs_block_pack_launch(hns_grid* g, const float* div, const float* src, float* dst, float dx, float omega, bool src_is_zero,
                                                                                 const hns::PackMirror* m, void* stream, bool* done, int iterations);
extern "C" __attribute__((visibility("hidden"))) bool hns_rbgs_block_packable(hns_grid* g);
extern "C" __attribute__((visibility("hidden"))) int hns_rbgs_block_mirror_launch(hns_grid* g, const float* div, const float* src, float* dst, float dx, float omega, bool src_is_zero,
                                                                                   const hns::PhaseMirror* m, void* stream, int iterations);
extern "C" __attribute__((visibility("hidden"))) int hns_chain_divergence(hns_grid* g, const float* vel3, float* div, float inv_dx, const hns::PhaseMirror* m, void* stream);
extern "C" __attribute__((visibility("hidden"))) int hns_chain_subtract_pressure_gradient(hns_grid* g, const float* vel3, const float* p, float* out3, float inv_dx,
                                                                                          const hns::PhaseMirror* m, void* stream);

extern "C" __attribute__((visibility("hidden"))) int hns_divergence_combust_buoyancy(hns_grid* g, const float* vel3, float* div, float inv_dx, const float* fuel, const float* waste,
                                                                                      const float* temperature, const float* flame, float* q4, float* vel3_out, float temp_gain,
                                                                                      float expansion, float dt, float ambient, float strength, void* stream);
extern "C" __attribute__((visibility("hidden"))) int hns_advect_scalars_q4(hns_grid* g, const float* vel3, const float* q4, float* const* q4_out, const float* const* in,
                                                                            float* const* out, int n, float dt, float inv_dx, void* stream);
extern "C" __attribute__((visibility("hidden"))) bool hns_advect_q4_ok(const hns_grid* g);

extern "C" __attribute__((visibility("hidden"))) int hns_combustion_div(const float* fuel, const float* waste, float* divergence, float expansion, uint64_t n,
                                                                        void* stream);
extern "C" __attribute__((visibility("hidden"))) int hns_combustion_fields(const float* fuel, const float* waste, const float* temperature, const float* flame,
                                                                           float* out_fuel, float* out_waste, float* out_temperature, float* out_flame,
                                                                           float temp_gain, uint64_t n, void* stream);

extern "C" __attribute__((visibility("hidden"))) int hns_arena_get(size_t need, int device, void** p, size_t* bytes);
extern "C" __attribute__((visibility("hidden"))) void hns_arena_put(void* p, size_t bytes, int device);

int hns_grid_upload(hns_grid* g);
void hns_grid_free_device(hns_grid* g);
int hns_grid_upload_schedule(hns_grid* g);
int hns_grid_build_blocks(hns_grid* g);
void hns_grid_retire_blocks(hns_grid* g);
int hns_rbgs_block_shape(hns_grid* g, int* k_max);
bool hns_rbgs_block_lean(hns_grid* g, int lb, int k);
int hns_rbgs_block_launch(hns_grid* g, int lb, int k, bool src_is_zero, const float* div, const float* src, float* dst, float dx2, float omega, void* stream);
int hns_grid_host_tables(const hns_grid* g);
```

### hnanosolver_amd/csrc/hns_regrid.hip

```cpp
#include <algorithm>
#include <cstring>
#include <memory>
#include <type_traits>
#include <vector>

#include "hns_device.hpp"
#include "hns_dilate.hpp"

typedef int v4i_act __attribute__((ext_vector_type(4)));
typedef float v3f_act __attribute__((ext_vector_type(3)));
__device__ float hns_act_load_f32(v4i_act rsrc, int voffset, int soffset, int aux) __asm("llvm.amdgcn.raw.buffer.load.f32");
__device__ v3f_act hns_act_load_v3f32(v4i_act rsrc, int voffset, int soffset, int aux) __asm("llvm.amdgcn.raw.buffer.load.v3f32");

namespace hns {
namespace {

constexpr unsigned long long kEmptySlot = ~0ull;
constexpr uint64_t kMaxCandidates = uint64_t(1) << 23;
constexpr int kCopyFields = 16;
constexpr uint32_t kSdfFill = 0x01010101u;

__device__ __forceinline__ void load_mask(const unsigned char* masks, int l, uint64_t (&m)[8]) {
	const uint64_t* w = masks ? (const uint64_t*)(masks + 64 * (size_t)l) : nullptr;
#pragma unroll
// ... 488 lines not shown
		HNS_HIP(hipEventRecord(s->rev[2], st));
		return HNS_OK;
	}

	int masks() {
		HNS_TRY(scratch.carve([&](auto&& slice) { slice(map, 4 * n_new); }));
		HNS_TRY(scratch.get(64 * n_new, &new_masks));
		if (!srcs.empty())
			HNS_TRY(scratch.carve([&](auto&& slice) {
				for (Source& q : srcs) slice(q.idx, 4 * n_new);
			}));
		for (size_t i = 0; i < srcs.size(); ++i) {
			Source& q = srcs[i];
			if (q.kind == Source::kVelocity) continue;
			HNS_HIP(hipMemsetAsync(q.idx, 0xFF, 4 * n_new, st));
			if (!q.l.n_leaves) continue;
			k_regrid_src_index<<<(unsigned)((q.l.n_leaves + 255) / 256), 256, 0, st>>>(ng->dev(), q.origins, (int)q.l.n_leaves, q.idx, dup + i);
			HNS_HIP(hipGetLastError());
		}
		const SrcHash vh{vsrc ? vsrc->origins : nullptr, vsrc ? vsrc->table : nullptr, vsrc ? vsrc->mask : 0u};
		k_regrid_masks<<<(unsigned)((n_new + 3) / 4), 256, 0, st>>>(s->grid->dev(), s->d_masks, (const int4*)ng->d_origins, (int)n_new, p, R, sdf ? sdf->idx : nullptr,
		                                                           sdf ? sdf->masks : nullptr, vh, vsrc ? vsrc->masks : nullptr, (uint64_t*)new_masks, map,
		                                                           vsrc ? vsrc->idx : nullptr);
		HNS_HIP(hipGetLastError());
		HNS_HIP(hipEventRecord(s->rev[3], st));
		return HNS_OK;
	}

	void field(FieldSet& fs, int j, const float* old, float* dst, const Source* q, uint32_t fill) const {
		const bool from_sdf = q && q->kind == Source::kSdf, add = q && !from_sdf;
		fs.a[j] = (const float4*)(from_sdf ? q->values : old), fs.map_a[j] = from_sdf ? q->idx : map;
		fs.b[j] = add ? (const float4*)q->values : nullptr, fs.map_b[j] = add ? q->idx : nullptr;
		fs.dst[j] = (float4*)dst, fs.fill[j] = fill;
	}

	int fields() {
		hns_sim shell;
		shell.names = s->names;
		HNS_TRY(scratch.get(hns_sim_arena_need(s, n_new * 512u), &new_fields));
		hns_sim_layout(&shell, new_fields, n_new * 512u);
		std::vector<const Source*> src_of(s->names.size(), nullptr);
		for (const Source& q : srcs)
			if (q.field >= 0) src_of[(size_t)q.field] = &q;
		const int i_sdf = s->find("collision_sdf");
		FieldSet fs{};
		field(fs, 0, s->vel, shell.vel, vsrc, 0u);
		HNS_TRY(launch_fields(fs, 1, 3, vsrc != nullptr, n_new, st));
		for (const bool add : {false, true}) {
			int nf = 0;
			for (size_t f = 0; f < s->names.size(); ++f) {
				const Source* q = src_of[f];
				if ((q && q->kind == Source::kFloat) != add) continue;
				field(fs, nf++, s->cur[f], shell.cur[f], q, (int)f == i_sdf ? kSdfFill : 0u);
				if (nf == kCopyFields) {
					HNS_TRY(launch_fields(fs, nf, 1, add, n_new, st));
					nf = 0;
				}
			}
			HNS_TRY(launch_fields(fs, nf, 1, add, n_new, st));
		}
		HNS_HIP(hipEventRecord(s->rev[4], st));
		return HNS_OK;
	}

	int commit(hns_grid** out) {
		std::vector<int> dups(srcs.size(), 0);
		if (!srcs.empty()) HNS_HIP(hipMemcpyAsync(dups.data(), dup, 4 * srcs.size(), hipMemcpyDeviceToHost, st));
		HNS_HIP(hipStreamSynchronize(st));
		for (size_t i = 0; i < srcs.size(); ++i) {
			if (!dups[i]) continue;
			if (srcs[i].kind == Source::kSdf)
				set_error("%s: duplicate SDF leaf origin", who);
			else
				set_error("%s: source %d ('%s'): duplicate leaf origin", who, srcs[i].index, srcs[i].name());
			return HNS_ERR_TOPOLOGY;
		}
		scratch.held.emplace_back(s->arena, s->arena_bytes);
		if (s->d_masks) scratch.held.emplace_back(s->d_masks, s->masks_bytes);
		s->arena = new_fields, s->arena_bytes = scratch.keep(new_fields);
		hns_sim_layout(s, new_fields, n_new * 512u);
		s->d_masks = (unsigned char*)new_masks, s->masks_bytes = scratch.keep(new_masks);
		s->grid = ng.release();
		s->forget();
		s->regrid_timed = true;
		*out = s->grid;
		return HNS_OK;
	}
};

int regrid(hns_sim* s, int p, const hns_leaf_source* src, int n_src, const hns_leaf_source& sdf, hipStream_t st, hns_grid** out, const char* who) {
	const hns_grid* og = s->grid;
	if (og->first_active != 0 || og->n_active != (uint64_t)og->topo.n_leaves) {
		set_error("%s: the grid's launch range is not the whole grid (a multi-GPU rank's grid cannot be regridded)", who);
		return HNS_ERR_INVALID_ARGUMENT;
	}
	DeviceScope on(s->device);
	Regrid r(s, p, st, who);
	HNS_TRY(r.sources(sdf, src, n_src));
	if (!s->rev[0])
		for (hipEvent_t& e : s->rev) HNS_HIP(hipEventCreate(&e));
	s->regrid_timed = false;
	HNS_TRY(r.candidates());
	HNS_TRY(r.order());
	HNS_TRY(r.masks());
	HNS_TRY(r.fields());
	return r.commit(out);
}


struct ActField {
	const float* p;
	float tol;
	int ncomp;
};
constexpr int kActRows = 16;
struct ActRows {
	ActField f[kActRows];
};

__global__ __launch_bounds__(64) void k_deactivate_table(ActRows rows, int n, ActField* dst, unsigned long long* count) {
	if ((int)threadIdx.x < n) dst[threadIdx.x] = rows.f[threadIdx.x];
	if (count && threadIdx.x == 0) *count = 0;
}

constexpr int kActSkip = 0x40000000;

__device__ __forceinline__ v4i_act leaf_rsrc(const float* p, unsigned bytes) {
	const unsigned long long a = (unsigned long long)p;
	v4i_act r;
	r.x = __builtin_amdgcn_readfirstlane((int)(unsigned)a);
	r.y = __builtin_amdgcn_readfirstlane((int)((unsigned)(a >> 32) & 0xffffu));
	r.z = (int)bytes;
	r.w = 0x00020000;
	return r;
}

__device__ __forceinline__ uint64_t readlane64(uint64_t v, int lane) {
	const uint32_t lo = (uint32_t)__builtin_amdgcn_readlane((int)(uint32_t)v, lane), hi = (uint32_t)__builtin_amdgcn_readlane((int)(uint32_t)(v >> 32), lane);
	return (uint64_t)hi << 32 | lo;
}

__global__ __launch_bounds__(256) void k_deactivate(const ActField* __restrict__ tab, int n_tab, const uint64_t* masks_in, uint64_t* masks_out, uint64_t n_leaves,
                                                    unsigned long long* count) {
	const uint64_t leaf = (uint64_t)blockIdx.x * 4 + (threadIdx.x >> 6);
	if (leaf >= n_leaves) return;
	const int lane = (int)(threadIdx.x & 63);
	const uint64_t word = masks_in && lane < 8 ? masks_in[8 * leaf + (uint64_t)lane] : ~0ull;
	uint64_t old[8], pend[8];
#pragma unroll
	for (int k = 0; k < 8; ++k) pend[k] = old[k] = readlane64(word, k);
	for (int f = 0; f < n_tab; ++f) {
		const ActField e = tab[f];
		if (e.ncomp == 1) {
			const v4i_act r = leaf_rsrc(e.p + 512 * leaf, 2048u);
			float x[8];
#pragma unroll
			for (int k = 0; k < 8; ++k) x[k] = hns_act_load_f32(r, pend[k] ? 4 * (64 * k + lane) : kActSkip, 0, 0);
#pragma unroll
			for (int k = 0; k < 8; ++k) pend[k] &= __ballot(fabsf(x[k]) <= e.tol);
		} else {
			const v4i_act r = leaf_rsrc(e.p + 1536 * leaf, 6144u);
			v3f_act x[8];
#pragma unroll
			for (int k = 0; k < 8; ++k) x[k] = hns_act_load_v3f32(r, pend[k] ? 12 * (64 * k + lane) : kActSkip, 0, 0);
#pragma unroll
			for (int k = 0; k < 8; ++k) pend[k] &= __ballot(fabsf(x[k].x) <= e.tol && fabsf(x[k].y) <= e.tol && fabsf(x[k].z) <= e.tol);
		}
		if (!(pend[0] | pend[1] | pend[2] | pend[3] | pend[4] | pend[5] | pend[6] | pend[7])) break;
	}
	uint64_t mine = 0;
	unsigned pop = 0;
#pragma unroll
	for (int k = 0; k < 8; ++k) {
		const uint64_t w = old[k] & ~pend[k];
		pop += (unsigned)__popcll(w);
		if (lane == k) mine = w;
	}
	if (lane < 8) masks_out[8 * leaf + (uint64_t)lane] = mine;
	if (count && lane == 0 && pop) atomicAdd(count, (unsigned long long)pop | 1ull << 40);
}

}
}

using namespace hns;

extern "C" int hns_sim_set_active_masks(hns_sim* s, const unsigned char* masks, void* stream) {
	if (!s) return fail(HNS_ERR_INVALID_ARGUMENT, "hns_sim_set_active_masks: null sim");
	const uint64_t n_leaves = s->n / 512u;
	if (!masks) {
		if (s->d_masks) hns_arena_put(s->d_masks, s->masks_bytes, s->device);
		s->d_masks = nullptr, s->masks_bytes = 0;
		return HNS_OK;
	}
	if (!n_leaves) return HNS_OK;
	if (!s->d_masks) {
		void* p = nullptr;
		size_t got = 0;
		HNS_TRY(hns_arena_get(64 * n_leaves, s->device, &p, &got));
		s->d_masks = (unsigned char*)p, s->masks_bytes = got;
	}
	HNS_HIP(hipMemcpyAsync(s->d_masks, masks, 64 * n_leaves, hipMemcpyHostToDevice, (hipStream_t)stream));
	return HNS_OK;
}

extern "C" int hns_sim_active_masks(hns_sim* s, unsigned char* out, void* stream) {
	if (!s || !out) return fail(HNS_ERR_INVALID_ARGUMENT, "hns_sim_active_masks: null argument");
	const uint64_t n_leaves = s->n / 512u;
	if (!s->d_masks) {
		memset(out, 0xFF, 64 * n_leaves);
		return HNS_OK;
	}
	HNS_HIP(hipMemcpyAsync(out, s->d_masks, 64 * n_leaves, hipMemcpyDeviceToHost, (hipStream_t)stream));
	HNS_HIP(hipStreamSynchronize((hipStream_t)stream));
	return HNS_OK;
}

namespace {
hns_grid* regrid_entry(hns_sim* s, int padding_voxels, const hns_leaf_source* sources, int n_sources, const int32_t* sdf_origins, uint64_t n_sdf,
                       const unsigned char* sdf_masks, const float* sdf_values, void* stream, int* err, const char* who) {
	int rc = HNS_OK;
	hns_grid* g = nullptr;
	if (!s || !s->grid || padding_voxels < 0 || padding_voxels > 1024 || (n_sdf && (!sdf_origins || !sdf_values))) {
		set_error("%s: bad arguments", who);
		rc = HNS_ERR_INVALID_ARGUMENT;
	} else if (s->cached) {
		set_error("%s: the sim belongs to a grid's cook cache", who);
		rc = HNS_ERR_INVALID_ARGUMENT;
	} else {
		const hns_leaf_source sdf{"collision_sdf", 1, sdf_origins, n_sdf, sdf_masks, sdf_values};
		rc = regrid(s, padding_voxels, sources, n_sources, sdf, (hipStream_t)stream, &g, who);
	}
	if (err) *err = rc;
	return rc == HNS_OK ? g : nullptr;
}
}

extern "C" hns_grid* hns_sim_regrid(hns_sim* s, int padding_voxels, const int32_t* sdf_origins, uint64_t n_sdf, const unsigned char* sdf_masks, const float* sdf_values,
                                    void* stream, int* err) {
	return regrid_entry(s, padding_voxels, nullptr, 0, sdf_origins, n_sdf, sdf_masks, sdf_values, stream, err, "hns_sim_regrid");
}

extern "C" hns_grid* hns_sim_regrid_sourced(hns_sim* s, int padding_voxels, const hns_leaf_source* sources, int n_sources, const int32_t* sdf_origins, uint64_t n_sdf,
                                            const unsigned char* sdf_masks, const float* sdf_values, void* stream, int* err) {
	return regrid_entry(s, padding_voxels, sources, n_sources, sdf_origins, n_sdf, sdf_masks, sdf_values, stream, err, "hns_sim_regrid_sourced");
}

extern "C" int hns_sim_regrid_times(hns_sim* s, float* ms4) {
	if (!s || !ms4) return fail(HNS_ERR_INVALID_ARGUMENT, "hns_sim_regrid_times: null argument");
	if (!s->regrid_timed) return fail(HNS_ERR_RUNTIME, "hns_sim_regrid_times: no regrid has completed on this sim");
	for (int i = 0; i < 4; ++i) HNS_HIP(hipEventElapsedTime(&ms4[i], s->rev[i], s->rev[i + 1]));
	return HNS_OK;
}

extern "C" int hns_sim_deactivate(hns_sim* s, const hns_activity_field* fields, int n_fields, uint64_t* counts, void* stream) {
	const char* who = "hns_sim_deactivate";
	if (!s || !s->grid) return fail(HNS_ERR_INVALID_ARGUMENT, "hns_sim_deactivate: null sim");
	if (s->cached) return fail(HNS_ERR_INVALID_ARGUMENT, "hns_sim_deactivate: the sim belongs to a grid's cook cache");
	std::vector<int> field_of;
	HNS_TRY(check_activity_fields(s, fields, n_fields, who, &field_of));
	const uint64_t n_leaves = s->n / 512u;
	if (!n_leaves) {
		if (counts) counts[0] = counts[1] = 0;
		return HNS_OK;
	}
	DeviceScope on(s->device);
	const hipStream_t st = (hipStream_t)stream;
	if (!s->d_act) {
		void* p = nullptr;
		size_t got = 0;
		HNS_TRY(hns_arena_get(16 + sizeof(ActField) * (s->names.size() + 1), s->device, &p, &got));
		s->d_act = p, s->act_bytes = got;
	}
	unsigned long long* d_count = (unsigned long long*)s->d_act;
	ActField* d_tab = (ActField*)((char*)s->d_act + 16);
	unsigned char* masks = s->d_masks;
	size_t masks_bytes = s->masks_bytes;
	if (!masks) {
		void* p = nullptr;
		HNS_TRY(hns_arena_get(64 * n_leaves, s->device, &p, &masks_bytes));
		masks = (unsigned char*)p;
	}
	int rc = HNS_OK;
	for (int i0 = 0; i0 < n_fields && rc == HNS_OK; i0 += kActRows) {
		ActRows rows{};
		const int n = std::min(kActRows, n_fields - i0);
		for (int j = 0; j < n; ++j) {
			const int f = field_of[(size_t)(i0 + j)];
			rows.f[j] = ActField{f < 0 ? s->vel : s->cur[(size_t)f], fields[i0 + j].tolerance, fields[i0 + j].ncomp};
		}
		k_deactivate_table<<<1, 64, 0, st>>>(rows, n, d_tab + i0, counts && i0 == 0 ? d_count : nullptr);
		if (hipGetLastError() != hipSuccess) rc = fail(HNS_ERR_HIP, "hns_sim_deactivate: table launch failed");
	}
	if (rc == HNS_OK) {
		k_deactivate<<<(unsigned)((n_leaves + 3) / 4), 256, 0, st>>>(d_tab, n_fields, (const uint64_t*)s->d_masks, (uint64_t*)masks, n_leaves,
		                                                            counts ? d_count : nullptr);
		if (hipGetLastError() != hipSuccess) rc = fail(HNS_ERR_HIP, "hns_sim_deactivate: kernel launch failed");
	}
	if (rc != HNS_OK) {
		if (masks != s->d_masks) hns_arena_put(masks, masks_bytes, s->device);
		return rc;
	}
	s->d_masks = masks, s->masks_bytes = masks_bytes;
	if (counts) {
		unsigned long long packed = 0;
		HNS_HIP(hipMemcpyAsync(&packed, d_count, sizeof(packed), hipMemcpyDeviceToHost, st));
		HNS_HIP(hipStreamSynchronize(st));
		counts[0] = packed & ((1ull << 40) - 1), counts[1] = packed >> 40;
	}
	return HNS_OK;
}
```

### hnanosolver_amd/csrc/hns_topology.cpp

```cpp
#include <cstdlib>
#include <cstring>
#include <thread>

#include "hns_internal.hpp"

namespace hns {

static thread_local std::string g_last_error;

void set_error(const char* fmt, ...) {
	char buf[1024];
	va_list ap;
	va_start(ap, fmt);
	vsnprintf(buf, sizeof(buf), fmt, ap);
	va_end(ap);
	g_last_error = buf;
}

Options& options() {
	static Options o;
	return o;
}

uint32_t hash_origin(int32_t x, int32_t y, int32_t z) {
	uint32_t h = (uint32_t)(x >> 3) * 0x9E3779B1u;
	h ^= (uint32_t)(y >> 3) * 0x85EBCA77u;
	h ^= (uint32_t)(z >> 3) * 0xC2B2AE3Du;
	h ^= h >> 15;
	h *= 0x2C1B3C6Du;
	h ^= h >> 12;
	return h;
}

int64_t Topology::find_leaf(int32_t ox, int32_t oy, int32_t oz) const {
	if (n_leaves == 0) return -1;
	uint32_t s = hash_origin(ox, oy, oz) & hash_mask;
	for (;;) {
		const int32_t l = hash[s];
		if (l < 0) return -1;
		const int32_t* o = &origins[4 * (size_t)l];
		if (o[0] == ox && o[1] == oy && o[2] == oz) return l;
		s = (s + 1) & hash_mask;
	}
}

uint64_t Topology::offset(int32_t i, int32_t j, int32_t k) const {
	const int64_t l = find_leaf(i & ~7, j & ~7, k & ~7);
	if (l < 0) return 0;
	return (uint64_t)l * 512u + (uint64_t)(((i & 7) << 6) | ((j & 7) << 3) | (k & 7)) + 1u;
}

int Topology::prepare(const int32_t* leaf_origins_xyz, int64_t n) {
	if (n < 0 || n > (int64_t(1) << 22)) {
		set_error("hns_grid: %lld leaves exceeds the 2^22-leaf (2^31-voxel) limit of 32-bit voxel indices", (long long)n);
		return HNS_ERR_TOPOLOGY;
	}
	n_leaves = n;
	have_tables = false;
	origins.assign((size_t)n * 4, 0);
	uint32_t size = 16;
	while ((int64_t)size < 2 * n + 2) size <<= 1;
	hash_mask = size - 1;
	for (int64_t l = 0; l < n; ++l) {
		const int32_t ox = leaf_origins_xyz[3 * l], oy = leaf_origins_xyz[3 * l + 1], oz = leaf_origins_xyz[3 * l + 2];
		if ((ox & 7) || (oy & 7) || (oz & 7)) {
			set_error("hns_grid: leaf %lld origin (%d,%d,%d) is not 8-aligned: coordinates are not leaf-dense", (long long)l, ox, oy, oz);
			return HNS_ERR_TOPOLOGY;
		}
		origins[4 * l] = ox;
		origins[4 * l + 1] = oy;
		origins[4 * l + 2] = oz;
	}
	return HNS_OK;
}

int Topology::build_tables() {
	const int64_t n = n_leaves;
	hash.assign((size_t)hash_mask + 1, -1);
	for (int64_t l = 0; l < n; ++l) {
		const int32_t ox = origins[4 * l], oy = origins[4 * l + 1], oz = origins[4 * l + 2];
		uint32_t s = hash_origin(ox, oy, oz) & hash_mask;
		while (hash[s] >= 0) {
			const int32_t* o = &origins[4 * (size_t)hash[s]];
			if (o[0] == ox && o[1] == oy && o[2] == oz) {
				set_error("hns_grid: leaf origin (%d,%d,%d) appears twice (leaves %d and %lld)", ox, oy, oz, hash[s], (long long)l);
				return HNS_ERR_TOPOLOGY;
			}
			s = (s + 1) & hash_mask;
		}
		hash[s] = (int32_t)l;
	}
	nbr27.assign((size_t)n * 27, -1);
	for (int64_t l = 0; l < n; ++l) {
		const int32_t* o = &origins[4 * (size_t)l];
		for (int dx = -1; dx <= 1; ++dx)
			for (int dy = -1; dy <= 1; ++dy)
				for (int dz = -1; dz <= 1; ++dz) {
					const int64_t nx = (int64_t)o[0] + 8 * dx, ny = (int64_t)o[1] + 8 * dy, nz = (int64_t)o[2] + 8 * dz;
					int64_t nb = -1;
					if (nx >= INT32_MIN && nx <= INT32_MAX && ny >= INT32_MIN && ny <= INT32_MAX && nz >= INT32_MIN && nz <= INT32_MAX)
						nb = find_leaf((int32_t)nx, (int32_t)ny, (int32_t)nz);
					nbr27[(size_t)l * 27 + (dx + 1) * 9 + (dy + 1) * 3 + (dz + 1)] = (int32_t)nb;
				}
	}
	have_tables = true;
	return HNS_OK;
}

}

using namespace hns;

extern "C" {

const char* hns_last_error(void) { return g_last_error.c_str(); }
int hns_version(void) { return HNS_VERSION; }

namespace {
struct OptionDesc {
	const char* name;
	std::atomic<int> Options::*field;
	const char* const* words;
};
const char* const kWordsRbgs[] = {"auto", "color", nullptr};
const char* const kWordsAdvect[] = {"auto", "generic", nullptr};
const char* const kWordsStencil[] = {"auto", "block", nullptr};
const char* const kWordsSchedule[] = {"auto", "linear", nullptr};
const char* const kWordsBool[] = {"0", "1", nullptr};
const char* const kWordsMirror[] = {"0", "1", "guarded", nullptr};
const char* const kWordsUnsplit[] = {"0", "1", "always", nullptr};
const char* const kWordsDivergence[] = {"auto", "row", "coalesced", "zpair", nullptr};
const OptionDesc kOptions[] = {
    {"rbgs", &Options::rbgs, kWordsRbgs},
    {"advect", &Options::advect_generic, kWordsAdvect},
    {"stencil", &Options::stencil_block, kWordsStencil},
    {"schedule", &Options::schedule, kWordsSchedule},
    {"cook_cache", &Options::cook_cache, kWordsBool},
    {"cook_pipeline", &Options::cook_pipeline, kWordsBool},
    {"divergence", &Options::divergence_form, kWordsDivergence},
    {"fuse", &Options::fuse_pointwise, kWordsBool},
    {"sor_block_lb", &Options::sor_block_lb, nullptr},
    {"dist_wire_us", &Options::dist_wire_us, nullptr},
    {"dist_mirror", &Options::dist_mirror, kWordsMirror},
    {"dist_unsplit", &Options::dist_unsplit, kWordsUnsplit},
};
const Options kDefaults;
}

int hns_set_option(const char* name, const char* value) {
	if (!name) return fail(HNS_ERR_INVALID_ARGUMENT, "hns_set_option: null name");
	for (const OptionDesc& d : kOptions) {
		if (strcmp(d.name, name) != 0) continue;
		if (!value) {
			(options().*d.field).store((kDefaults.*d.field).load());
			return HNS_OK;
		}
		if (!d.words) {
			char* end = nullptr;
			const long v = strtol(value, &end, 10);
			if (end == value || *end || v < 0 || v > 1 << 20) break;
			(options().*d.field).store((int)v);
			return HNS_OK;
		}
		for (int i = 0; d.words[i]; ++i)
			if (strcmp(d.words[i], value) == 0) {
				(options().*d.field).store(i);
				return HNS_OK;
			}
		break;
	}
	set_error("hns_set_option: unknown option or value: %s = %s", name, value ? value : "(default)");
	return HNS_ERR_INVALID_ARGUMENT;
}

const char* hns_get_option(const char* name) {
	static thread_local char buf[16];
	if (!name) return nullptr;
	for (const OptionDesc& d : kOptions) {
		if (strcmp(d.name, name) != 0) continue;
		const int v = (options().*d.field).load();
		if (d.words) return d.words[v];
		snprintf(buf, sizeof(buf), "%d", v);
		return buf;
	}
	return nullptr;
}

static hns_grid* grid_from_origins(const int32_t* origins, uint64_t n_leaves, float voxel_size, unsigned flags, int* err) {
	int rc = HNS_OK;
	hns_grid* g = new hns_grid;
	g->voxel_size = voxel_size;
	rc = g->topo.prepare(origins, (int64_t)n_leaves);
	if (rc == HNS_OK) {
		g->n_active = n_leaves;
		rc = (flags & HNS_GRID_HOST_ONLY) ? g->topo.build_tables() : hns_grid_upload(g);
	}
	if (rc != HNS_OK) {
		hns_grid_free_device(g);
		delete g;
		g = nullptr;
	}
	if (err) *err = rc;
	return g;
}

hns_grid* hns_grid_create_from_leaves(const int32_t* leaf_origins_xyz, uint64_t n_leaves, float voxel_size, unsigned flags, int* err) {
	if (!leaf_origins_xyz && n_leaves) {
		if (err) *err = fail(HNS_ERR_INVALID_ARGUMENT, "hns_grid_create_from_leaves: null origin array");
		return nullptr;
	}
	return grid_from_origins(leaf_origins_xyz, n_leaves, voxel_size, flags, err);
}

static int scan_coords(const char* who, const int32_t* coords, uint64_t n_voxels, unsigned flags, std::vector<int32_t>& origins) {
	if (!coords && n_voxels) {
		set_error("%s: null coordinate array", who);
		return HNS_ERR_INVALID_ARGUMENT;
	}
	if (n_voxels % 512u) {
		set_error("%s: %llu coordinates is not a multiple of 512: the domain must be leaf-dense", who, (unsigned long long)n_voxels);
		return HNS_ERR_TOPOLOGY;
	}
	const uint64_t n_leaves = n_voxels / 512u;
	origins.resize((size_t)n_leaves * 3);
	const bool validate = !(flags & HNS_GRID_SKIP_VALIDATE);
	unsigned n_threads = 1;
	if (validate && n_leaves >= 2048) {
		n_threads = std::thread::hardware_concurrency();
		if (n_threads == 0) n_threads = 1;
		if (n_threads > 16) n_threads = 16;
	}
	std::vector<uint64_t> first_bad(n_threads, UINT64_MAX);
	auto scan = [&](unsigned t) {
		const uint64_t l0 = n_leaves * t / n_threads, l1 = n_leaves * (t + 1) / n_threads;
		for (uint64_t l = l0; l < l1; ++l) {
			const int32_t* c = coords + 3 * 512 * l;
			origins[3 * l] = c[0];
			origins[3 * l + 1] = c[1];
			origins[3 * l + 2] = c[2];
			if (!validate || first_bad[t] != UINT64_MAX) continue;
			for (int n = 1; n < 512; ++n) {
				const int32_t* v = c + 3 * n;
				if (v[0] != c[0] + (n >> 6) || v[1] != c[1] + ((n >> 3) & 7) || v[2] != c[2] + (n & 7)) {
					first_bad[t] = 512 * l + n;
					break;
				}
			}
		}
	};
	if (n_threads == 1) {
		scan(0);
	} else {
		std::vector<std::thread> pool;
		for (unsigned t = 1; t < n_threads; ++t) pool.emplace_back(scan, t);
		scan(0);
		for (auto& th : pool) th.join();
	}
	for (unsigned t = 0; t < n_threads; ++t) {
		if (first_bad[t] == UINT64_MAX) continue;
		const uint64_t i = first_bad[t];
		const int32_t* v = coords + 3 * i;
		set_error("%s: coordinate %llu = (%d,%d,%d) breaks the leaf-dense x<<6|y<<3|z order of leaf %llu", who, (unsigned long long)i, v[0], v[1], v[2],
		          (unsigned long long)(i / 512));
		return HNS_ERR_TOPOLOGY;
	}
	return HNS_OK;
}

hns_grid* hns_grid_create(const int32_t* coords, uint64_t n_voxels, float voxel_size, unsigned flags, int* err) {
	std::vector<int32_t> origins;
	const int rc = scan_coords("hns_grid_create", coords, n_voxels, flags, origins);
	if (rc != HNS_OK) {
		if (err) *err = rc;
		return nullptr;
	}
	return grid_from_origins(origins.data(), n_voxels / 512u, voxel_size, flags, err);
}

int hns_grid_matches(const hns_grid* g, const int32_t* coords, uint64_t n_voxels, unsigned flags) {
	if (!g) return fail(HNS_ERR_INVALID_ARGUMENT, "hns_grid_matches: null grid");
	std::vector<int32_t> origins;
	const int rc = scan_coords("hns_grid_matches", coords, n_voxels, flags, origins);
	if (rc != HNS_OK) return rc;
	const uint64_t n_leaves = n_voxels / 512u;
	if (n_leaves != (uint64_t)g->topo.n_leaves) return 0;
	for (uint64_t l = 0; l < n_leaves; ++l) {
		const int32_t* o = &g->topo.origins[4 * (size_t)l];
		if (o[0] != origins[3 * l] || o[1] != origins[3 * l + 1] || o[2] != origins[3 * l + 2]) return 0;
	}
	return 1;
}

void hns_grid_destroy(hns_grid* g) {
	if (!g) return;
	hns_grid_free_device(g);
	delete g;
}

uint64_t hns_grid_leaf_count(const hns_grid* g) { return g ? (uint64_t)g->topo.n_leaves : 0; }
uint64_t hns_grid_voxel_count(const hns_grid* g) { return g ? (uint64_t)g->topo.n_leaves * 512u : 0; }
float hns_grid_voxel_size(const hns_grid* g) { return g ? g->voxel_size : 0.0f; }
uint64_t hns_grid_active_leaves(const hns_grid* g) { return g ? g->n_active : 0; }

int hns_grid_set_active_range(hns_grid* g, uint64_t first, uint64_t count) {
	if (!g) return fail(HNS_ERR_INVALID_ARGUMENT, "hns_grid_set_active_range: null grid");
	if (first > (uint64_t)g->topo.n_leaves || count > (uint64_t)g->topo.n_leaves - first)
		return fail(HNS_ERR_INVALID_ARGUMENT, "hns_grid_set_active_range: range beyond the grid's leaves");
	g->first_active = count ? first : 0;
	g->n_active = count;
	return g->on_device ? hns_grid_upload_schedule(g) : HNS_OK;
}

int hns_grid_set_active_leaves(hns_grid* g, uint64_t n_active) {
	if (!g) return fail(HNS_ERR_INVALID_ARGUMENT, "hns_grid_set_active_leaves: null grid");
	if (n_active > (uint64_t)g->topo.n_leaves) return fail(HNS_ERR_INVALID_ARGUMENT, "hns_grid_set_active_leaves: more active leaves than leaves");
	return hns_grid_set_active_range(g, 0, n_active);
}

int hns_grid_set_outside_element(hns_grid* g, uint64_t element_index) {
	if (!g) return fail(HNS_ERR_INVALID_ARGUMENT, "hns_grid_set_outside_element: null grid");
	if (element_index >= (uint64_t)g->topo.n_leaves * 512u && element_index != 0)
		return fail(HNS_ERR_INVALID_ARGUMENT, "hns_grid_set_outside_element: index beyond the grid");
	g->outside_element = element_index;
	return HNS_OK;
}

int hns_grid_offsets(const hns_grid* g, const int32_t* ijk, uint64_t n, uint64_t* out) {
	if (!g || (!ijk && n) || (!out && n)) return fail(HNS_ERR_INVALID_ARGUMENT, "hns_grid_offsets: null argument");
	if (int rc = hns_grid_host_tables(g)) return rc;
	for (uint64_t t = 0; t < n; ++t) out[t] = g->topo.offset(ijk[3 * t], ijk[3 * t + 1], ijk[3 * t + 2]);
	return HNS_OK;
}

int hns_grid_neighbor_table(const hns_grid* g, int32_t* out) {
	if (!g || !out) return fail(HNS_ERR_INVALID_ARGUMENT, "hns_grid_neighbor_table: null argument");
	if (int rc = hns_grid_host_tables(g)) return rc;
	memcpy(out, g->topo.nbr27.data(), g->topo.nbr27.size() * sizeof(int32_t));
	return HNS_OK;
}

int hns_grid_coords(const hns_grid* g, int32_t* out) {
	if (!g || !out) return fail(HNS_ERR_INVALID_ARGUMENT, "hns_grid_coords: null argument");
	for (int64_t l = 0; l < g->topo.n_leaves; ++l) {
		const int32_t* o = &g->topo.origins[4 * (size_t)l];
		for (int n = 0; n < 512; ++n) {
			int32_t* c = out + 3 * (l * 512 + n);
			c[0] = o[0] + (n >> 6);
			c[1] = o[1] + ((n >> 3) & 7);
			c[2] = o[2] + (n & 7);
		}
	}
	return HNS_OK;
}

}
```

### hnanosolver_amd/device.py

```python
from __future__ import annotations

import ctypes as C
from typing import List, Optional, Sequence

import numpy as np

from . import _lib, leafio
from ._lib import hns_combustion_params, hns_field, lib
from .api import CombustionParams, IndexGridHandle, _raise, create_grid_from_leaves


def _torch():
    import torch

    return torch


def _ptr(t) -> int:
    if t is None:
        return 0
    if not t.is_cuda:
        raise RuntimeError("hnanosolver_amd.device: tensor is not on a HIP device (there is no CPU fallback)")
    if t.dtype != _torch().float32 and t.dtype != _torch().int32:
        raise TypeError("expected float32 / int32 tensor")
    if not t.is_contiguous():
        raise TypeError("expected a contiguous tensor")
    return t.data_ptr()


def current_stream() -> int:
    return int(_torch().cuda.current_stream().cuda_stream)


def advect_vector(grid: IndexGridHandle, u, out, dt: float, inv_dx: float, sdf=None, has_collision: bool = False):
    _raise(lib.hns_dev_advect_vector(grid.ptr, _ptr(u), _ptr(out), _ptr(sdf), int(has_collision), dt, inv_dx, current_stream()))
    return out


def advect_scalar(grid: IndexGridHandle, u, src, dst, dt: float, inv_dx: float, sdf=None, has_collision: bool = False):
    _raise(lib.hns_dev_advect_scalar(grid.ptr, _ptr(u), _ptr(src), _ptr(dst), _ptr(sdf), int(has_collision), dt, inv_dx, current_stream()))
    return dst


def advect_scalars(grid: IndexGridHandle, u, srcs: Sequence, dsts: Sequence, dt: float, inv_dx: float, sdf=None, has_collision: bool = False):
    n = len(srcs)
    ins = (C.c_void_p * max(1, n))(*[_ptr(t) for t in srcs])
    outs = (C.c_void_p * max(1, n))(*[_ptr(t) for t in dsts])
    _raise(lib.hns_dev_advect_scalars(grid.ptr, _ptr(u), ins, outs, n, _ptr(sdf), int(has_collision), dt, inv_dx, current_stream()))
    return dsts


def divergence(grid: IndexGridHandle, u, div, inv_dx: float):
    _raise(lib.hns_dev_divergence(grid.ptr, _ptr(u), _ptr(div), inv_dx, current_stream()))
    return div


def rbgs_color(grid: IndexGridHandle, div, p, dx: float, omega: float, color: int):
    _raise(lib.hns_dev_rbgs_color(grid.ptr, _ptr(div), _ptr(p), dx, omega, color, current_stream()))
    return p


def rbgs_iterate(grid: IndexGridHandle, div, p_a, p_b, dx: float, omega: float, iterations: int):
    in_b = C.c_int(0)
    _raise(lib.hns_dev_rbgs_iterate(grid.ptr, _ptr(div), _ptr(p_a), _ptr(p_b), dx, omega, iterations, C.byref(in_b), current_stream()))
    return p_b if in_b.value else p_a


def rbgs_plan(grid: IndexGridHandle, iterations: int):
    buf = C.create_string_buffer(256)
    n, k = C.c_int(0), C.c_int(0)
    _raise(lib.hns_grid_rbgs_plan(grid.ptr, iterations, buf, 256, C.byref(n), C.byref(k)))
    return buf.value.decode(), n.value, k.value


def time_rbgs(grid: IndexGridHandle, div, p_a, p_b, dx: float, omega: float, iterations: int, reps: int) -> float:
    ms = C.c_float(0.0)
    _raise(lib.hns_dev_time_rbgs(grid.ptr, _ptr(div), _ptr(p_a), _ptr(p_b), dx, omega, iterations, reps, C.byref(ms), current_stream()))
    return float(ms.value)


def subtract_pressure_gradient(grid: IndexGridHandle, u, p, out, inv_dx: float, sdf=None, has_collision: bool = False):
    _raise(lib.hns_dev_subtract_pressure_gradient(grid.ptr, _ptr(u), _ptr(p), _ptr(out), _ptr(sdf), int(has_collision), inv_dx, current_stream()))
    return out


def combustion_oxygen(fuel, waste, temperature, div, flame, out_fuel, out_waste, out_temperature, out_flame, temp_gain: float, expansion: float):
    _raise(lib.hns_dev_combustion_oxygen(_ptr(fuel), _ptr(waste), _ptr(temperature), _ptr(div), _ptr(flame), _ptr(out_fuel), _ptr(out_waste),
                                         _ptr(out_temperature), _ptr(out_flame), temp_gain, expansion, fuel.numel(), current_stream()))


def temperature_buoyancy(u, temperature, out, dt: float, ambient: float, strength: float):
    _raise(lib.hns_dev_temperature_buoyancy(_ptr(u), _ptr(temperature), _ptr(out), dt, ambient, strength, temperature.numel(), current_stream()))
    return out


def vorticity_confinement(grid: IndexGridHandle, u, out, dt: float, inv_dx: float, scale: float, factor_scale: float):
    _raise(lib.hns_dev_vorticity_confinement(grid.ptr, _ptr(u), _ptr(out), dt, inv_dx, scale, factor_scale, current_stream()))
    return out


def enforce_collision_boundaries(grid: IndexGridHandle, u, sdf, voxel_size: float):
    _raise(lib.hns_dev_enforce_collision_boundaries(grid.ptr, _ptr(u), _ptr(sdf), voxel_size, current_stream()))
    return u


def pack_leaves(field, leaf_ids, packed, ncomp: int = 1):
    _raise(lib.hns_dev_pack_leaves(_ptr(field), _ptr(leaf_ids), leaf_ids.numel(), _ptr(packed), ncomp, current_stream()))
    return packed


def unpack_leaves(packed, leaf_ids, field, ncomp: int = 1):
    _raise(lib.hns_dev_unpack_leaves(_ptr(packed), _ptr(leaf_ids), leaf_ids.numel(), _ptr(field), ncomp, current_stream()))
    return field


def _leaf_source(entry, leaves, need, keep, ncomp: Optional[int] = None) -> None:
    so, sm, sv = leaves
    o = np.ascontiguousarray(so, dtype=np.int32).reshape(-1, 3)
    v = np.ascontiguousarray(sv, dtype=np.float32)
    nc = ncomp or (3 if (v.ndim == 2 and v.shape[1] == 3) else 1)
    if v.size != len(o) * 512 * nc:
        per_leaf = "512" if ncomp else f"512 x {nc}"
        raise ValueError(f"{need[0]} {len(o)} x {per_leaf} floats, got {v.size}")
    m = None if sm is None else np.ascontiguousarray(sm, dtype=np.uint8).reshape(-1)
    if m is not None and m.size != len(o) * 64:
        raise ValueError(f"{need[1]} {len(o)} x 64 bytes, got {m.size}")
    keep += [o, m, v]
    entry.ncomp, entry.origins, entry.n_leaves, entry.values = nc, o.ctypes.data, len(o), v.ctypes.data
    entry.masks = None if m is None else m.ctypes.data


class Sim:

    def __init__(self, grid: IndexGridHandle, float_names: Sequence[str]):
        self.grid = grid
        self.names = list(float_names)
        arr = (C.c_char_p * max(1, len(self.names)))(*[n.encode() for n in self.names])
        err = C.c_int(0)
        self._ptr = lib.hns_sim_create(grid.ptr, arr, len(self.names), C.byref(err))
        if not self._ptr:
            _raise(err.value if err.value < 0 else _lib.HNS_ERR_RUNTIME)

    def _fields(self, arrays: dict):
        arr = (hns_field * max(1, len(arrays)))()
        keep = []
        for i, (name, a) in enumerate(arrays.items()):
            if a.dtype != np.float32 or not a.flags["C_CONTIGUOUS"]:
                raise TypeError(f"{name}: need C-contiguous float32")
            b = name.encode()
            keep.append(b)
            arr[i].name = b
            arr[i].ncomp = 3 if (a.ndim == 2 and a.shape[1] == 3) else 1
            arr[i].host = a.ctypes.data_as(C.POINTER(C.c_float))
        return arr, len(arrays), keep

    def upload(self, arrays: dict, stream: Optional[int] = None) -> None:
        arr, n, keep = self._fields(arrays)
        _raise(lib.hns_sim_upload(self._ptr, arr, n, stream or 0))

    def download(self, arrays: dict, stream: Optional[int] = None) -> None:
        arr, n, keep = self._fields(arrays)
        _raise(lib.hns_sim_download(self._ptr, arr, n, stream or 0))

    def substep(self, iterations: int, dt: float, voxel_size: float, params: CombustionParams, has_collision: bool = False, stream: int = 0) -> None:
        p = params._c()
        _raise(lib.hns_sim_substep(self._ptr, iterations, dt, voxel_size, C.byref(p), int(has_collision), stream))

    def core_substep(self, iterations: int, dt: float, voxel_size: float, stream: int = 0) -> None:
        _raise(lib.hns_sim_core_substep(self._ptr, iterations, dt, voxel_size, stream))

    def pressure_solve(self, iterations: int, voxel_size: float, stream: int = 0) -> None:
        _raise(lib.hns_sim_pressure_solve(self._ptr, iterations, voxel_size, stream))

    def timing(self, max_solves: int) -> None:
        _raise(lib.hns_sim_timing(self._ptr, max_solves))

    def pressure_time(self):
        ms, n = C.c_float(0.0), C.c_longlong(0)
        _raise(lib.hns_sim_pressure_time(self._ptr, C.byref(ms), C.byref(n)))
        return float(ms.value), int(n.value)

    def stage_timing(self, max_substeps: int) -> None:
        _raise(lib.hns_sim_stage_timing(self._ptr, max_substeps))

    def stage_times(self):
        ms, n = (C.c_float * 5)(), C.c_longlong(0)
        _raise(lib.hns_sim_stage_times(self._ptr, ms, C.byref(n)))
        return dict(zip(("advect_vector", "divergence", "pressure", "gradient", "advect_scalars"), [float(x) for x in ms])), int(n.value)

    def set_active_masks(self, masks: Optional[np.ndarray], stream: int = 0) -> None:
        if masks is None:
            _raise(lib.hns_sim_set_active_masks(self._ptr, None, stream))
            return
        m = np.ascontiguousarray(masks, dtype=np.uint8)
        if m.size != self.grid.leaf_count() * 64:
            raise ValueError(f"masks: need {self.grid.leaf_count()} x 64 bytes, got {m.size}")
        _raise(lib.hns_sim_set_active_masks(self._ptr, m.ctypes.data, stream))

    def active_masks(self, stream: int = 0) -> np.ndarray:
        out = np.empty((self.grid.leaf_count(), 64), dtype=np.uint8)
        _raise(lib.hns_sim_active_masks(self._ptr, out.ctypes.data, stream))
        return out

    def regrid(self, padding: int, sdf=None, sources=None, stream: int = 0) -> IndexGridHandle:
        err, keep = C.c_int(0), []
        sdf_e = _lib.hns_leaf_source()
        if sdf is not None:
            _leaf_source(sdf_e, sdf, ("sdf values: need", "sdf masks: need"), keep, 1)
        sdf_args = (sdf_e.origins, sdf_e.n_leaves, sdf_e.masks, sdf_e.values)
        if sources is None:
            ptr = lib.hns_sim_regrid(self._ptr, int(padding), *sdf_args, stream, C.byref(err))
        else:
            arr = (_lib.hns_leaf_source * max(1, len(sources)))()
            for i, (name, leaves) in enumerate(sources.items()):
                keep.append(name.encode())
                arr[i].name = keep[-1]
                _leaf_source(arr[i], leaves, (f"source {name}: need", f"source {name}: masks need"), keep)
            ptr = lib.hns_sim_regrid_sourced(self._ptr, int(padding), arr, len(sources), *sdf_args, stream, C.byref(err))
        if not ptr:
            _raise(err.value if err.value < 0 else _lib.HNS_ERR_RUNTIME)
        self.grid = IndexGridHandle(ptr)
        return self.grid

    def deactivate(self, tolerances: dict, velocity: Optional[float] = None, counts: bool = False, stream: int = 0):
        arr, n = leafio.activity_fields(tolerances, velocity)
        out = (C.c_uint64 * 2)()
        _raise(lib.hns_sim_deactivate(self._ptr, arr, n, out if counts else None, stream))
        return (int(out[0]), int(out[1])) if counts else None

    def regrid_times(self):
        ms = (C.c_float * 4)()
        _raise(lib.hns_sim_regrid_times(self._ptr, ms))
        return dict(zip(("candidates", "host", "masks", "fields"), [float(x) for x in ms]))

    def close(self) -> None:
        if self._ptr:
            lib.hns_sim_destroy(self._ptr)
            self._ptr = 0

    def __del__(self):
        try:
            self.close()
        except Exception:
            pass
```

### include/hns.h

```cpp
#ifndef HNS_H
#define HNS_H

#include <stdint.h>

#ifdef __cplusplus
extern "C" {
#endif

#define HNS_VERSION 100

#define HNS_OK 0
#define HNS_ERR_INVALID_ARGUMENT (-1)
#define HNS_ERR_RUNTIME (-2)
#define HNS_ERR_HIP (-3)
#define HNS_ERR_NO_DEVICE (-4)
#define HNS_ERR_TOPOLOGY (-5)

const char* hns_last_error(void);
int hns_version(void);
int hns_device_count(void);
int hns_trim_memory(void);
int hns_set_option(const char* name, const char* value);
const char* hns_get_option(const char* name);


typedef struct hns_grid hns_grid;

#define HNS_GRID_DEFAULT 0u
#define HNS_GRID_HOST_ONLY 1u
#define HNS_GRID_SKIP_VALIDATE 2u

hns_grid* hns_grid_create(const int32_t* coords_xyz, uint64_t n_voxels, float voxel_size, unsigned flags, int* err);
hns_grid* hns_grid_create_from_leaves(const int32_t* leaf_origins_xyz, uint64_t n_leaves, float voxel_size, unsigned flags, int* err);
void hns_grid_destroy(hns_grid*);

uint64_t hns_grid_leaf_count(const hns_grid*);
uint64_t hns_grid_voxel_count(const hns_grid*);
float hns_grid_voxel_size(const hns_grid*);
int hns_grid_set_active_leaves(hns_grid*, uint64_t n_active);
int hns_grid_set_active_range(hns_grid*, uint64_t first, uint64_t count);
uint64_t hns_grid_active_leaves(const hns_grid*);
int hns_grid_set_outside_element(hns_grid*, uint64_t element_index);
int hns_grid_offsets(const hns_grid*, const int32_t* ijk, uint64_t n, uint64_t* out);
int hns_grid_neighbor_table(const hns_grid*, int32_t* out);
int hns_grid_coords(const hns_grid*, int32_t* out_xyz);
int hns_grid_matches(const hns_grid*, const int32_t* coords_xyz, uint64_t n_voxels, unsigned flags);
int hns_grid_release_cache(hns_grid*);
int hns_grid_export_nanovdb(const hns_grid*, void* buffer, uint64_t capacity, uint64_t* size_out);
int hns_grid_launch_tables(const hns_grid*, int32_t* sched);


#define HNS_FILL_ZERO 0
#define HNS_FILL_SDF 1
int hns_gather_leaves(const int32_t* domain_origins, uint64_t n_domain, const int32_t* src_origins, uint64_t n_src, const float* src_values, int ncomp, int fill,
                      float* out);
int hns_scatter_leaves(const float* flat, uint64_t n_domain, int ncomp, float* const* leaf_buffers);
int hns_dilate_leaves(const int32_t* origins, uint64_t n, const unsigned char* active_masks, int padding_voxels, int32_t* out_origins, uint64_t capacity,
                      uint64_t* n_out);
int hns_dilate_leaf_masks(const int32_t* origins, uint64_t n, const unsigned char* active_masks, int padding_voxels, int32_t* out_origins,
                          unsigned char* out_masks, uint64_t capacity, uint64_t* n_out);
int hns_union_leaves(const int32_t* a, uint64_t na, const int32_t* b, uint64_t nb, int32_t* out_origins, uint64_t capacity, uint64_t* n_out);
int hns_add_leaves(const int32_t* a_origins, uint64_t na, const unsigned char* a_masks, const float* a_values, const int32_t* b_origins, uint64_t nb,
                   const unsigned char* b_masks, const float* b_values, int ncomp, int32_t* out_origins, unsigned char* out_masks, float* out_values,
                   uint64_t capacity, uint64_t* n_out);
typedef struct {
	const char* name;
	int ncomp;
	float tolerance;
} hns_activity_field;
int hns_deactivate_leaf_masks(uint64_t n_leaves, const unsigned char* masks_in, const hns_activity_field* fields, const float* const* values, int n_fields,
                              unsigned char* masks_out, uint64_t* counts);


typedef struct {
	const char* name;
	int ncomp;
	float* host;
} hns_field;

typedef struct {
	float expansionRate, temperatureRelease, buoyancyStrength, ambientTemp, vorticityScale, factorScale;
} hns_combustion_params;

int hns_compute_sim(hns_grid*, hns_field* fields, int n_fields, int iterations, float dt, float voxel_size,
                    const hns_combustion_params* params, int has_collision, void* stream);
int hns_compute_sim_resident(hns_grid*, hns_field* fields, int n_fields, const unsigned char* resident, int* uploads_skipped, int iterations, float dt,
                             float voxel_size, const hns_combustion_params* params, int has_collision, void* stream);
int hns_advect_index_grid(hns_grid*, hns_field* fields, int n_fields, float dt, float voxel_size, void* stream);
int hns_advect_index_grid_velocity(hns_grid*, hns_field* fields, int n_fields, float dt, float voxel_size, void* stream);
int hns_project_non_divergent(hns_grid*, hns_field* fields, int n_fields, uint64_t iterations, float voxel_size, void* stream);
int hns_divergence(hns_grid*, hns_field* fields, int n_fields, float voxel_size, void* stream);


typedef struct hns_sim hns_sim;

hns_sim* hns_sim_create(hns_grid*, const char* const* float_names, int n_float, int* err);
void hns_sim_destroy(hns_sim*);
int hns_sim_upload(hns_sim*, const hns_field* fields, int n_fields, void* stream);
int hns_sim_download(hns_sim*, hns_field* fields, int n_fields, void* stream);
int hns_sim_substep(hns_sim*, int iterations, float dt, float voxel_size, const hns_combustion_params*, int has_collision, void* stream);
int hns_sim_core_substep(hns_sim*, int iterations, float dt, float voxel_size, void* stream);
int hns_sim_pressure_solve(hns_sim*, int iterations, float voxel_size, void* stream);
int hns_sim_timing(hns_sim*, int max_solves);
int hns_sim_pressure_time(hns_sim*, float* total_ms, long long* launches);
int hns_sim_stage_timing(hns_sim*, int max_substeps);
int hns_sim_stage_times(hns_sim*, float* ms5, long long* substeps);
float* hns_sim_velocity_ptr(hns_sim*);
float* hns_sim_field_ptr(hns_sim*, const char* name);
float* hns_sim_divergence_ptr(hns_sim*);
float* hns_sim_pressure_ptr(hns_sim*);


int hns_sim_set_active_masks(hns_sim*, const unsigned char* masks, void* stream);
int hns_sim_active_masks(hns_sim*, unsigned char* out, void* stream);
hns_grid* hns_sim_regrid(hns_sim*, int padding_voxels, const int32_t* sdf_origins, uint64_t n_sdf, const unsigned char* sdf_masks,
                         const float* sdf_values, void* stream, int* err);
int hns_sim_regrid_times(hns_sim*, float* ms4);
typedef struct {
	const char* name;
	int ncomp;
	const int32_t* origins;
	uint64_t n_leaves;
	const unsigned char* masks;
	const float* values;
} hns_leaf_source;
hns_grid* hns_sim_regrid_sourced(hns_sim*, int padding_voxels, const hns_leaf_source* sources, int n_sources, const int32_t* sdf_origins, uint64_t n_sdf,
                                 const unsigned char* sdf_masks, const float* sdf_values, void* stream, int* err);
int hns_sim_deactivate(hns_sim*, const hns_activity_field* fields, int n_fields, uint64_t* counts, void* stream);


int hns_dev_advect_vector(hns_grid*, const float* vel3, float* out3, const float* sdf, int has_collision, float dt, float inv_dx, void* stream);
int hns_dev_advect_scalar(hns_grid*, const float* vel3, const float* in, float* out, const float* sdf, int has_collision, float dt, float inv_dx,
                          void* stream);
int hns_dev_advect_scalars(hns_grid*, const float* vel3, const float* const* in, float* const* out, int n, const float* sdf, int has_collision,
                           float dt, float inv_dx, void* stream);
int hns_dev_divergence(hns_grid*, const float* vel3, float* div, float inv_dx, void* stream);
int hns_dev_rbgs_color(hns_grid*, const float* div, float* p, float dx, float omega, int color, void* stream);
int hns_dev_rbgs_iterate(hns_grid*, const float* div, float* p_a, float* p_b, float dx, float omega, int iterations, int* result_in_b,
                         void* stream);
int hns_dev_subtract_pressure_gradient(hns_grid*, const float* vel3, const float* p, float* out3, const float* sdf, int has_collision, float inv_dx,
                                       void* stream);
int hns_dev_combustion_oxygen(const float* fuel, const float* waste, const float* temperature, float* divergence, const float* flame,
                              float* out_fuel, float* out_waste, float* out_temperature, float* out_flame, float temp_gain, float expansion,
                              uint64_t n, void* stream);
int hns_dev_temperature_buoyancy(const float* vel3, const float* temperature, float* out3, float dt, float ambient, float strength, uint64_t n,
                                 void* stream);
int hns_dev_vorticity_confinement(hns_grid*, const float* vel3, float* out3, float dt, float inv_dx, float confinement_scale, float factor_scale,
                                  void* stream);
int hns_dev_enforce_collision_boundaries(hns_grid*, float* vel3, const float* sdf, float voxel_size, void* stream);

int hns_dev_pack_leaves(const float* field, const int32_t* leaf_ids, uint64_t n, float* packed, int ncomp, void* stream);
int hns_dev_unpack_leaves(const float* packed, const int32_t* leaf_ids, uint64_t n, float* field, int ncomp, void* stream);


typedef struct hns_dist hns_dist;

typedef struct {
	int world, rank, peers, sweeps_per_exchange;
	uint64_t boundary_leaves, interior_leaves, ghost_leaves;
	uint64_t region_voxels_sent[4];
	uint64_t bytes_sent[4];
	uint64_t messages_sent, exchanges;
	uint64_t halo_peers;
	uint64_t packed_exchanges;
	uint64_t chained;
} hns_dist_stats;

#define HNS_DIST_DEFAULT 0u
#define HNS_DIST_PLAN_ONLY 1u
#define HNS_DIST_LEAF_ORDER 2u
hns_dist* hns_dist_create(const int32_t* global_leaf_origins_xyz, uint64_t n_leaves, int world, int rank, float voxel_size, int n_scalars,
                          int sweeps_per_exchange, unsigned flags, int* err);
void hns_dist_destroy(hns_dist*);
int hns_dist_unique_id(void* out128);
int hns_dist_connect_rccl(hns_dist*, const void* unique_id128);
#define HNS_DIST_IPC_BLOB_BYTES 2048
int hns_dist_ipc_export(hns_dist*, void* out_blob);
int hns_dist_connect_ipc(hns_dist*, const void* blobs_of_all_ranks);
int hns_dist_connect_local(hns_dist* const* ranks, int world);
int hns_dist_connect_loopback(hns_dist*);
int hns_dist_connect_loopback_rccl(hns_dist*);
uint64_t hns_dist_owned_leaves(const hns_dist*);
uint64_t hns_dist_first_owned_leaf(const hns_dist*);
int hns_dist_owned_leaf_ids(const hns_dist*, int64_t* out_global_ids);
int hns_dist_partition_axis(const hns_dist*);
int hns_dist_one_sided_sweeps(uint64_t n_leaves, int world);
int hns_dist_info(const hns_dist*, hns_dist_stats* out);
int hns_dist_local_leaves(const hns_dist*, int64_t* out_global_ids);
int hns_dist_peer_rank(const hns_dist*, int peer);
int hns_dist_peer_region(const hns_dist*, int peer, int type, int is_send, int32_t* leaves, unsigned char* masks, uint64_t* n_leaves, uint64_t* n_voxels);
int hns_dist_upload(hns_dist*, const float* vel3, const float* const* scalars, void* stream);
int hns_dist_download(hns_dist*, float* vel3, float* const* scalars, float* pressure, void* stream);
int hns_dist_download_local(hns_dist*, int which, float* out, void* stream);
int hns_dist_core_substep(hns_dist*, int iterations, float dt, void* stream);
int hns_dist_local_core_substep(hns_dist* const* ranks, int world, int iterations, float dt, void* stream);
int hns_dist_timing(hns_dist*, int max_solves);
int hns_dist_sim_substep(hns_dist*, int iterations, float dt, const hns_combustion_params*, const int* field_index, int has_collision, void* stream);
int hns_dist_local_sim_substep(hns_dist* const* ranks, int world, int iterations, float dt, const hns_combustion_params*, const int* field_index, int has_collision,
                               void* stream);
int hns_dist_pressure_time(hns_dist*, float* total_ms, long long* sweeps);
int hns_dist_synchronize(hns_dist*, void* stream);

int hns_dev_time_rbgs(hns_grid*, const float* div, float* p_a, float* p_b, float dx, float omega, int iterations, int reps, float* ms_per_launch,
                      void* stream);

int hns_grid_rbgs_plan(hns_grid*, int iterations, char* description, uint64_t description_bytes, int* launches, int* iterations_per_launch);

#ifdef __cplusplus
}
#endif
#endif
```

Measured before the change: 647.1.

## Fuse next-substep velocity advection into scalar advection kernel as look-ahead

The scalar advection kernel, which already reads the final velocity and stages it into shared memory, gains a variant that also computes the next substep's MacCormack-advected velocity and writes it to the adv buffer. The following substep's part_a then skips its separate vector-advection launch when the memo matches the grid, dt and voxel size. This saves one kernel launch and a full read of velocity per substep, at the cost of extra registers and shared memory in the scalar kernel. It also adds invalidation logic for regrid, external velocity access and graph capture.

```diff
diff --git a/hnanosolver_amd/_lib.py b/hnanosolver_amd/_lib.py
--- a/hnanosolver_amd/_lib.py
+++ b/hnanosolver_amd/_lib.py
@@ -106,6 +106,7 @@
     "hns_sim_pressure_time": (_i, [_vp, C.POINTER(C.c_float), C.POINTER(C.c_longlong)]),
     "hns_sim_stage_timing": (_i, [_vp, _i]),
     "hns_sim_stage_times": (_i, [_vp, C.POINTER(C.c_float), C.POINTER(C.c_longlong)]),
+    "hns_sim_lookahead_counts": (_i, [_vp, C.POINTER(C.c_longlong), C.POINTER(C.c_longlong)]),
     "hns_sim_velocity_ptr": (_vp, [_vp]),
     "hns_sim_field_ptr": (_vp, [_vp, C.c_char_p]),
     "hns_sim_divergence_ptr": (_vp, [_vp]),
@@ -119,6 +120,7 @@
     "hns_dev_advect_vector": (_i, [_vp, _fp, _fp, _fp, _i, _f, _f, _vp]),
     "hns_dev_advect_scalar": (_i, [_vp, _fp, _fp, _fp, _fp, _i, _f, _f, _vp]),
     "hns_dev_advect_scalars": (_i, [_vp, _fp, C.POINTER(C.c_void_p), C.POINTER(C.c_void_p), _i, _fp, _i, _f, _f, _vp]),
+    "hns_dev_advect_scalars_ahead": (_i, [_vp, _fp, C.POINTER(C.c_void_p), C.POINTER(C.c_void_p), _i, _fp, _f, _f, _vp]),
     "hns_dev_divergence": (_i, [_vp, _fp, _fp, _f, _vp]),
     "hns_dev_rbgs_color": (_i, [_vp, _fp, _fp, _f, _f, _i, _vp]),
     "hns_dev_rbgs_iterate": (_i, [_vp, _fp, _fp, _fp, _f, _f, _i, _ip, _vp]),
diff --git a/hnanosolver_amd/csrc/hns_advect.hip b/hnanosolver_amd/csrc/hns_advect.hip
--- a/hnanosolver_amd/csrc/hns_advect.hip
+++ b/hnanosolver_amd/csrc/hns_advect.hip
@@ -549,8 +549,10 @@
 	for (int q = 0; q < 8; ++q) ix[q] = T.t[perm[q]] < 0 ? oob : T.t[perm[q]];
 }
 
-template <bool Q4>
-__global__ __launch_bounds__(512) __attribute__((amdgpu_waves_per_eu(Q4 ? 6 : 4))) void k_advect_scalars_n(const GridDev g, const float* __restrict__ u, const ScalarPtrs P, const float scaled_dt) {
+template <bool Q4, bool AHEAD = false>
+__global__ __launch_bounds__(512) __attribute__((amdgpu_waves_per_eu(Q4 || AHEAD ? 6 : 4))) void k_advect_scalars_n(const GridDev g, const float* __restrict__ u, const ScalarPtrs P, const float scaled_dt,
+                                                                                                            float* __restrict__ adv_out) {
+	static_assert(!(Q4 && AHEAD), "the look-ahead form is float-only");
 	__shared__ int s_nbr[27];
 	__shared__ int s_base[27];
 	__shared__ unsigned s_b4[27];
@@ -593,41 +595,89 @@
 	const unsigned sx_ = (unsigned)(bi - (L.org.x - 1)), sy_ = (unsigned)(bj - (L.org.y - 1)), sz_ = (unsigned)(bk - (L.org.z - 1));
 	const bool bboxed = FIRST && max(sx_, max(sy_, sz_)) <= 8u;
 	const int ba = bboxed ? (int)((sx_ * 10u + sy_) * 10u + sz_) : 0;
-	{
-		float tx, ty, tz;
+	f3 vf = {0.0f, 0.0f, 0.0f};
+	__shared__ float s_vbox[AHEAD ? 3 * kVP : 1];
+	__shared__ float s_wf[AHEAD ? 3 * 512 : 1];
+	if constexpr (AHEAD) {
+		const int obv = ((n >> 6) + 1) * kVX + (((n >> 3) & 7) + 1) * kVY + (n & 7) + 1;
+		s_vbox[obv] = vc.x, s_vbox[obv + kVP] = vc.y, s_vbox[obv + 2 * kVP] = vc.z;
+		f3 hv = {0.0f, 0.0f, 0.0f};
+		int vcell = 0;
+		if (n < kBoxShell) {
+			int slot, local;
+			box_shell_entry<kVX, kVY>(n, slot, local, vcell);
+			hv = ldv(ru, s_b4[slot] + ((unsigned)local << 2));
+		}
+		const TapsB T = make_taps_b(g, s_nbr, s_b4p, L.org, bx, by, bz);
+		V3 c[8];
+#pragma unroll
+		for (int q = 0; q < 8; ++q) {
+			const v3f v = hns_buffer_load_v3f32(ru, (int)(T.o[perm[q]] + (T.o[perm[q]] << 1)), 0, 0);
+			c[perm[q]].xy = v2f32{v.x, v.y};
+			c[perm[q]].z = v.z;
+		}
+		const float* __restrict__ uoob = u + 3 * (size_t)g.oob;
+		const f3 uo = {uoob[0], uoob[1], uoob[2]};
+		if (n < kBoxShell) s_vbox[vcell] = hv.x, s_vbox[vcell + kVP] = hv.y, s_vbox[vcell + 2 * kVP] = hv.z;
+		{
+			const float tx = T.fx, ty = T.fy, tz = T.fz;
+			const float itx = 1.0f - tx, ity = 1.0f - ty, itz = 1.0f - tz;
+			const float w00 = itx * ity, w10 = tx * ity, w01 = itx * ty, w11 = tx * ty;
+			bw[0] = w00 * itz, bw[1] = w10 * itz, bw[2] = w01 * itz, bw[3] = w11 * itz, bw[4] = w00 * tz, bw[5] = w10 * tz, bw[6] = w01 * tz, bw[7] = w11 * tz;
+		}
+		V3 z[4];
+#pragma unroll
+		for (int q = 0; q < 8; ++q) {
+			const int t = perm[q];
+			const bool outside = T.o[t] >= kOutside;
+			bo[q] = outside ? oob4 : T.o[t];
+			const float tx = outside ? uo.x : c[t].xy.x, ty = outside ? uo.y : c[t].xy.y, tz = outside ? uo.z : c[t].z;
+			vf.x = vf.x + bw[q] * tx;
+			vf.y = vf.y + bw[q] * ty;
+			vf.z = vf.z + bw[q] * tz;
+			if (t & 1) z[t >> 1] = lerp_v3(c[t - 1], c[t], T.fz);
+		}
+		{
+			const V3 y0 = lerp_v3(z[0], z[1], T.fy), y1 = lerp_v3(z[2], z[3], T.fy);
+			const V3 r = lerp_v3(y0, y1, T.fx);
+			s_wf[n] = r.xy.x, s_wf[n + 512] = r.xy.y, s_wf[n + 1024] = r.z;
+		}
+	} else {
+		{
+			float tx, ty, tz;
+			if (bboxed) {
+				tx = bx - (float)bi, ty = by - (float)bj, tz = bz - (float)bk;
+#pragma unroll
+				for (int q = 0; q < 8; ++q) bo[q] = 0u;
+			} else {
+				const TapsB T = make_taps_b(g, s_nbr, s_b4p, L.org, bx, by, bz);
+				tx = T.fx, ty = T.fy, tz = T.fz;
+#pragma unroll
+				for (int q = 0; q < 8; ++q) bo[q] = T.o[perm[q]] >= kOutside ? oob4 : T.o[perm[q]];
+			}
+			const float itx = 1.0f - tx, ity = 1.0f - ty, itz = 1.0f - tz;
+			const float w00 = itx * ity, w10 = tx * ity, w01 = itx * ty, w11 = tx * ty;
+			bw[0] = w00 * itz, bw[1] = w10 * itz, bw[2] = w01 * itz, bw[3] = w11 * itz, bw[4] = w00 * tz, bw[5] = w10 * tz, bw[6] = w01 * tz, bw[7] = w11 * tz;
+		}
+		f3 vt[8];
+		if (!bboxed) {
+#pragma unroll
+			for (int q = 0; q < 8; ++q) vt[q] = ldv(ru, bo[q]);
+		}
+		if constexpr (FIRST) __syncthreads();
 		if (bboxed) {
-			tx = bx - (float)bi, ty = by - (float)bj, tz = bz - (float)bk;
-#pragma unroll
-			for (int q = 0; q < 8; ++q) bo[q] = 0u;
-		} else {
-			const TapsB T = make_taps_b(g, s_nbr, s_b4p, L.org, bx, by, bz);
-			tx = T.fx, ty = T.fy, tz = T.fz;
-#pragma unroll
-			for (int q = 0; q < 8; ++q) bo[q] = T.o[perm[q]] >= kOutside ? oob4 : T.o[perm[q]];
-		}
-		const float itx = 1.0f - tx, ity = 1.0f - ty, itz = 1.0f - tz;
-		const float w00 = itx * ity, w10 = tx * ity, w01 = itx * ty, w11 = tx * ty;
-		bw[0] = w00 * itz, bw[1] = w10 * itz, bw[2] = w01 * itz, bw[3] = w11 * itz, bw[4] = w00 * tz, bw[5] = w10 * tz, bw[6] = w01 * tz, bw[7] = w11 * tz;
-	}
-	f3 vt[8];
-	if (!bboxed) {
-#pragma unroll
-		for (int q = 0; q < 8; ++q) vt[q] = ldv(ru, bo[q]);
-	}
-	if constexpr (FIRST) __syncthreads();
-	if (bboxed) {
+#pragma unroll
+			for (int q = 0; q < 8; ++q) {
+				const int a = ba + (q & 1) * 100 + ((q >> 1) & 1) * 10 + (q >> 2);
+				vt[q] = f3{s_ubox[a], s_ubox[a + kBox], s_ubox[a + 2 * kBox]};
+			}
+		}
 #pragma unroll
 		for (int q = 0; q < 8; ++q) {
-			const int a = ba + (q & 1) * 100 + ((q >> 1) & 1) * 10 + (q >> 2);
-			vt[q] = f3{s_ubox[a], s_ubox[a + kBox], s_ubox[a + 2 * kBox]};
-		}
-	}
-	f3 vf = {0.0f, 0.0f, 0.0f};
-#pragma unroll
-	for (int q = 0; q < 8; ++q) {
-		vf.x = vf.x + bw[q] * vt[q].x;
-		vf.y = vf.y + bw[q] * vt[q].y;
-		vf.z = vf.z + bw[q] * vt[q].z;
+			vf.x = vf.x + bw[q] * vt[q].x;
+			vf.y = vf.y + bw[q] * vt[q].y;
+			vf.z = vf.z + bw[q] * vt[q].z;
+		}
 	}
 	const float qx = bx + scaled_dt * vf.x, qy = by + scaled_dt * vf.y, qz = bz + scaled_dt * vf.z;
 	const int qi = __float2int_rd(qx), qj = __float2int_rd(qy), qk = __float2int_rd(qz);
@@ -736,6 +786,49 @@
 		mn = fminf(mn, phiF);
 		mx = fmaxf(mx, phiF);
 		P.out[s][idx] = fmaxf(mn, fminf(phiCorr, mx));
+	}
+	if constexpr (AHEAD) {
+		__syncthreads();
+		int m = n;
+		asm volatile("" : "+v"(m));
+		const int obv = ((m >> 6) + 1) * kVX + (((m >> 3) & 7) + 1) * kVY + (m & 7) + 1;
+		const float wx = (float)(L.org.x + (m >> 6)), wy = (float)(L.org.y + ((m >> 3) & 7)), wz = (float)(L.org.z + (m & 7));
+		const f3 vo = f3{s_vbox[obv], s_vbox[obv + kVP], s_vbox[obv + 2 * kVP]};
+		const f3 wf = f3{s_wf[m], s_wf[m + 512], s_wf[m + 1024]};
+		const float cx = wx - scaled_dt * vo.x, cy = wy - scaled_dt * vo.y, cz = wz - scaled_dt * vo.z;
+		const float sx = cx + scaled_dt * wf.x, sy = cy + scaled_dt * wf.y, sz = cz + scaled_dt * wf.z;
+		const int i = __float2int_rd(sx), j = __float2int_rd(sy), k = __float2int_rd(sz);
+		const unsigned ux = (unsigned)(i - (L.org.x - 1)), uy = (unsigned)(j - (L.org.y - 1)), uz = (unsigned)(k - (L.org.z - 1));
+		f3 wb;
+		if (__all(max(ux, max(uy, uz)) <= 8u)) {
+			wb = tri_v_box(s_vbox, (int)(ux * (unsigned)kVX + uy * (unsigned)kVY + uz), sx - (float)i, sy - (float)j, sz - (float)k);
+		} else {
+			const TapsB T2 = make_taps_b(g, s_nbr, s_b4p, L.org, sx, sy, sz);
+			wb = tri_v_b(ru, T2);
+		}
+		f3 wc = {wf.x + 0.5f * (vo.x - wb.x), wf.y + 0.5f * (vo.y - wb.y), wf.z + 0.5f * (vo.z - wb.z)};
+		const int ev[6] = {obv - kVX, obv + kVX, obv - kVY, obv + kVY, obv - 1, obv + 1};
+		f3 vmn = vo, vmx = vo;
+#pragma unroll
+		for (int d = 0; d < 6; ++d) {
+			const V3 t = box_v3(s_vbox, ev[d]);
+			vmn.x = fminf(vmn.x, t.xy.x);
+			vmx.x = fmaxf(vmx.x, t.xy.x);
+			vmn.y = fminf(vmn.y, t.xy.y);
+			vmx.y = fmaxf(vmx.y, t.xy.y);
+			vmn.z = fminf(vmn.z, t.z);
+			vmx.z = fmaxf(vmx.z, t.z);
+		}
+		vmn.x = fminf(vmn.x, wf.x);
+		vmx.x = fmaxf(vmx.x, wf.x);
+		vmn.y = fminf(vmn.y, wf.y);
+		vmx.y = fmaxf(vmx.y, wf.y);
+		vmn.z = fminf(vmn.z, wf.z);
+		vmx.z = fmaxf(vmx.z, wf.z);
+		wc.x = fmaxf(vmn.x, fminf(wc.x, vmx.x));
+		wc.y = fmaxf(vmn.y, fminf(wc.y, vmx.y));
+		wc.z = fmaxf(vmn.z, fminf(wc.z, vmx.z));
+		st3(adv_out, idx, wc);
 	}
 }
 
@@ -875,12 +968,38 @@
 		{
 			GridDev gd = g->dev();
 			gd.rev = 1;
-			hipLaunchKernelGGL(k_advect_scalars_n<false>, grid, block, 0, (hipStream_t)stream, gd, vel3, P, scaled_dt);
+			hipLaunchKernelGGL(k_advect_scalars_n<false>, grid, block, 0, (hipStream_t)stream, gd, vel3, P, scaled_dt, (float*)nullptr);
 		}
 		else
 			hipLaunchKernelGGL(k_advect_scalars<false>, grid, block, 0, (hipStream_t)stream, g->dev(), vel3, P, sdf, scaled_dt);
 	}
 	return launch_status("hns_dev_advect_scalars");
+}
+
+bool hns_advect_ahead_ok(const hns_grid* g) { return narrow_fields(g); }
+
+int hns_dev_advect_scalars_ahead(hns_grid* g, const float* vel3, const float* const* in, float* const* out, int n, float* adv_out3, float dt, float inv_dx, void* stream) {
+	if (int rc = check_grid(g, "hns_dev_advect_scalars_ahead")) return rc;
+	NULLCHK(!vel3 || !adv_out3 || (n > 0 && (!in || !out)), "hns_dev_advect_scalars_ahead");
+	if (vel3 == adv_out3) return fail(HNS_ERR_INVALID_ARGUMENT, "hns_dev_advect_scalars_ahead: adv_out3 must not alias vel3");
+	if (n < 0 || n > HNS_MAX_SCALARS) return fail(HNS_ERR_INVALID_ARGUMENT, "hns_dev_advect_scalars_ahead: between 0 and 8 fields");
+	if (!narrow_fields(g)) return fail(HNS_ERR_INVALID_ARGUMENT, "hns_dev_advect_scalars_ahead: grid too large for 32-bit offsets (or option advect = generic)");
+	if (g->n_active == 0) return HNS_OK;
+	ScalarPtrs P;
+	P.n = n;
+	P.q4 = nullptr, P.q4_out[0] = P.q4_out[1] = P.q4_out[2] = P.q4_out[3] = nullptr;
+	for (int s = 0; s < HNS_MAX_SCALARS; ++s) {
+		P.in[s] = s < n ? in[s] : nullptr;
+		P.out[s] = s < n ? out[s] : nullptr;
+		if (s < n && (!P.in[s] || !P.out[s])) {
+			set_error("hns_dev_advect_scalars_ahead: null device pointer for field %d", s);
+			return HNS_ERR_INVALID_ARGUMENT;
+		}
+	}
+	GridDev gd = g->dev();
+	gd.rev = 1;
+	hipLaunchKernelGGL((k_advect_scalars_n<false, true>), dim3((unsigned)g->n_active), dim3(512), 0, (hipStream_t)stream, gd, vel3, P, dt * inv_dx, adv_out3);
+	return launch_status("hns_dev_advect_scalars_ahead");
 }
 
 int hns_advect_scalars_q4(hns_grid* g, const float* vel3, const float* q4, float* const* q4_out, const float* const* in, float* const* out, int n, float dt, float inv_dx,
@@ -903,7 +1022,7 @@
 	}
 	GridDev gd = g->dev();
 	gd.rev = 1;
-	hipLaunchKernelGGL(k_advect_scalars_n<true>, dim3((unsigned)g->n_active), dim3(512), 0, (hipStream_t)stream, gd, vel3, P, dt * inv_dx);
+	hipLaunchKernelGGL(k_advect_scalars_n<true>, dim3((unsigned)g->n_active), dim3(512), 0, (hipStream_t)stream, gd, vel3, P, dt * inv_dx, (float*)nullptr);
 	return launch_status("hns_advect_scalars_q4");
 }
 
diff --git a/hnanosolver_amd/csrc/hns_api.hip b/hnanosolver_amd/csrc/hns_api.hip
--- a/hnanosolver_amd/csrc/hns_api.hip
+++ b/hnanosolver_amd/csrc/hns_api.hip
@@ -204,7 +204,17 @@
 	return HNS_OK;
 }
 
-extern "C" float* hns_sim_velocity_ptr(hns_sim* s) { return s ? s->vel : nullptr; }
+extern "C" float* hns_sim_velocity_ptr(hns_sim* s) {
+	if (!s) return nullptr;
+	s->ahead_off = true;
+	s->drop_ahead();
+	return s->vel;
+}
+extern "C" int hns_sim_lookahead_counts(hns_sim* s, long long* produced, long long* consumed) {
+	if (!s || !produced || !consumed) return fail(HNS_ERR_INVALID_ARGUMENT, "hns_sim_lookahead_counts: null argument");
+	*produced = s->ahead_produced, *consumed = s->ahead_consumed;
+	return HNS_OK;
+}
 extern "C" float* hns_sim_field_ptr(hns_sim* s, const char* name) {
 	if (!s || !name) return nullptr;
 	const int k = s->find(name);
@@ -274,7 +284,7 @@
 	return HNS_OK;
 }
 
-static int sim_advect_scalars(hns_sim* s, const float* sdf, bool coll, float dt, float inv_dx, void* stream) {
+static int sim_advect_scalars(hns_sim* s, const float* sdf, bool coll, float dt, float inv_dx, void* stream, bool* ahead) {
 	std::vector<const float*> ins;
 	std::vector<float*> outs;
 	std::vector<int> which;
@@ -284,13 +294,21 @@
 		outs.push_back(s->nxt[i]);
 		which.push_back((int)i);
 	}
-	HNS_TRY(hns_dev_advect_scalars(s->grid, s->vel, ins.data(), outs.data(), (int)ins.size(), sdf, coll, dt, inv_dx,
-	                               stream));
+	*ahead = *ahead && !coll && !ins.empty() && ins.size() <= 8 && hns_advect_ahead_ok(s->grid);
+	if (*ahead)
+		HNS_TRY(hns_dev_advect_scalars_ahead(s->grid, s->vel, ins.data(), outs.data(), (int)ins.size(), s->adv, dt, inv_dx, stream));
+	else
+		HNS_TRY(hns_dev_advect_scalars(s->grid, s->vel, ins.data(), outs.data(), (int)ins.size(), sdf, coll, dt, inv_dx, stream));
 	for (int i : which) std::swap(s->cur[i], s->nxt[i]);
 	return HNS_OK;
 }
 
 namespace {
+uint32_t float_bits(float x) {
+	uint32_t b;
+	memcpy(&b, &x, 4);
+	return b;
+}
 struct Substep {
 	hns_sim* s;
 	int iterations;
@@ -298,6 +316,7 @@
 	const hns_combustion_params* params;
 	int ci[4];
 	bool coll = false, fused = false;
+	bool ahead_live = false;
 	const float* sdf = nullptr;
 	void* stream;
 	hipEvent_t* stage_events = nullptr;
@@ -315,6 +334,16 @@
 		inv_dx = 1.0f / vs;
 		params = prm;
 		stream = st;
+		ahead_live = !s->ahead_off && options().lookahead.load() != kLookaheadOff;
+		if (ahead_live) {
+			hipStreamCaptureStatus cs = hipStreamCaptureStatusNone;
+			if (hipStreamIsCapturing((hipStream_t)stream, &cs) != hipSuccess) {
+				(void)hipGetLastError();
+				cs = hipStreamCaptureStatusActive;
+			}
+			if (cs != hipStreamCaptureStatusNone) ahead_live = false, s->ahead_off = true;
+		}
+		if (!ahead_live) s->drop_ahead();
 		if (!full()) return HNS_OK;
 		if (s->names.empty()) return fail(HNS_ERR_RUNTIME, "No float blocks found in input data.");
 		for (int c = 0; c < 4; ++c) {
@@ -336,8 +365,15 @@
 	int part_a() {
 		hns_grid* g = s->grid;
 		HNS_TRY(mark(0));
+		const hns_sim::Ahead& m = s->ahead;
+		const bool memo = ahead_live && !coll && m.valid && m.grid == g && m.first == g->first_active && m.n_active == g->n_active && m.dt_bits == float_bits(dt) &&
+		                  m.vs_bits == float_bits(voxel_size);
+		s->drop_ahead();
 		if (coll) HNS_TRY(hns_dev_enforce_collision_boundaries(g, s->vel, sdf, voxel_size, stream));
-		HNS_TRY(hns_dev_advect_vector(g, s->vel, s->adv, sdf, coll, dt, inv_dx, stream));
+		if (memo)
+			++s->ahead_consumed;
+		else
+			HNS_TRY(hns_dev_advect_vector(g, s->vel, s->adv, sdf, coll, dt, inv_dx, stream));
 		if (full() && (int)params->factorScale != 0) {
 			HNS_TRY(hns_dev_vorticity_confinement(g, s->adv, s->tmp, dt, inv_dx,
 			                                      params->vorticityScale, params->factorScale, stream));
@@ -372,7 +408,17 @@
 	}
 	int part_c() {
 		HNS_TRY(mark(4));
-		if (!fused) return sim_advect_scalars(s, sdf, coll, dt, inv_dx, stream);
+		const uint32_t dtb = float_bits(dt), vsb = float_bits(voxel_size);
+		bool ahead = ahead_live && !fused && (options().lookahead.load() == kLookaheadOn || (s->have_last && s->last_dt_bits == dtb && s->last_vs_bits == vsb));
+		s->have_last = true, s->last_dt_bits = dtb, s->last_vs_bits = vsb;
+		if (!fused) {
+			HNS_TRY(sim_advect_scalars(s, sdf, coll, dt, inv_dx, stream, &ahead));
+			if (ahead) {
+				s->ahead = hns_sim::Ahead{true, s->grid, s->grid->first_active, s->grid->n_active, dtb, vsb};
+				++s->ahead_produced;
+			}
+			return HNS_OK;
+		}
 		std::vector<const float*> ins;
 		std::vector<float*> outs;
 		float* q4_out[4];
@@ -479,6 +525,7 @@
 		}
 	}
 	if (guard.s) {
+		guard.s->ahead_off = true, guard.s->drop_ahead();
 		if (g->n_active != (uint64_t)g->topo.n_leaves) {
 			hns_sim* s = guard.s;
 			const size_t bytes = sizeof(float) * (size_t)s->n;
@@ -494,6 +541,7 @@
 	}
 	int err = HNS_OK;
 	guard.s = sim_create(g, names.data(), (int)names.size(), g->n_active != (uint64_t)g->topo.n_leaves, stream, &err);
+	if (guard.s) guard.s->ahead_off = true;
 	if (err != HNS_OK || !use_cache) return err;
 	std::lock_guard<std::mutex> lock(g->host_mutex);
 	if (g->sim_cache.size() >= 2) {
diff --git a/hnanosolver_amd/csrc/hns_internal.hpp b/hnanosolver_amd/csrc/hns_internal.hpp
--- a/hnanosolver_amd/csrc/hns_internal.hpp
+++ b/hnanosolver_amd/csrc/hns_internal.hpp
@@ -88,6 +88,7 @@
 
 enum { kRbgsAuto = 0, kRbgsColor = 1 };
 enum { kScheduleAuto = 0, kScheduleLinear = 1 };
+enum { kLookaheadAuto = 0, kLookaheadOff = 1, kLookaheadOn = 2 };
 struct Options {
 	std::atomic<int> rbgs{kRbgsAuto};
 	std::atomic<int> advect_generic{0};
@@ -97,6 +98,7 @@
 	std::atomic<int> cook_pipeline{1};
 	std::atomic<int> divergence_form{0};
 	std::atomic<int> fuse_pointwise{1};
+	std::atomic<int> lookahead{kLookaheadAuto};
 	std::atomic<int> sor_block_lb{0};
 	std::atomic<int> dist_wire_us{0};
 	std::atomic<int> dist_mirror{1};
@@ -215,7 +217,20 @@
 	Handed handed_vel;
 	std::vector<Handed> handed_cur;
 	static constexpr int kVelocity = -1, kEverything = -2;
+	struct Ahead {
+		bool valid = false;
+		const hns_grid* grid = nullptr;
+		uint64_t first = 0, n_active = 0;
+		uint32_t dt_bits = 0, vs_bits = 0;
+	};
+	Ahead ahead;
+	bool ahead_off = false;
+	bool have_last = false;
+	uint32_t last_dt_bits = 0, last_vs_bits = 0;
+	long long ahead_produced = 0, ahead_consumed = 0;
+	void drop_ahead() { ahead.valid = false; }
 	void forget(int k = kEverything) {
+		drop_ahead();
 		if (k == kEverything || k == kVelocity) handed_vel = Handed{};
 		for (size_t i = 0; i < handed_cur.size(); ++i)
 			if (k == kEverything || k == (int)i) handed_cur[i] = Handed{};
@@ -262,6 +277,7 @@
 extern "C" __attribute__((visibility("hidden"))) int hns_advect_scalars_q4(hns_grid* g, const float* vel3, const float* q4, float* const* q4_out, const float* const* in,
                                                                             float* const* out, int n, float dt, float inv_dx, void* stream);
 extern "C" __attribute__((visibility("hidden"))) bool hns_advect_q4_ok(const hns_grid* g);
+extern "C" __attribute__((visibility("hidden"))) bool hns_advect_ahead_ok(const hns_grid* g);
 
 extern "C" __attribute__((visibility("hidden"))) int hns_combustion_div(const float* fuel, const float* waste, float* divergence, float expansion, uint64_t n,
                                                                         void* stream);
diff --git a/hnanosolver_amd/csrc/hns_regrid.hip b/hnanosolver_amd/csrc/hns_regrid.hip
--- a/hnanosolver_amd/csrc/hns_regrid.hip
+++ b/hnanosolver_amd/csrc/hns_regrid.hip
@@ -814,6 +814,7 @@
 		return rc;
 	}
 	s->d_masks = masks, s->masks_bytes = masks_bytes;
+	s->drop_ahead();
 	if (counts) {
 		unsigned long long packed = 0;
 		HNS_HIP(hipMemcpyAsync(&packed, d_count, sizeof(packed), hipMemcpyDeviceToHost, st));
diff --git a/hnanosolver_amd/csrc/hns_topology.cpp b/hnanosolver_amd/csrc/hns_topology.cpp
--- a/hnanosolver_amd/csrc/hns_topology.cpp
+++ b/hnanosolver_amd/csrc/hns_topology.cpp
@@ -130,6 +130,7 @@
 const char* const kWordsMirror[] = {"0", "1", "guarded", nullptr};
 const char* const kWordsUnsplit[] = {"0", "1", "always", nullptr};
 const char* const kWordsDivergence[] = {"auto", "row", "coalesced", "zpair", nullptr};
+const char* const kWordsLookahead[] = {"auto", "0", "1", nullptr};
 const OptionDesc kOptions[] = {
     {"rbgs", &Options::rbgs, kWordsRbgs},
     {"advect", &Options::advect_generic, kWordsAdvect},
@@ -139,6 +140,7 @@
     {"cook_pipeline", &Options::cook_pipeline, kWordsBool},
     {"divergence", &Options::divergence_form, kWordsDivergence},
     {"fuse", &Options::fuse_pointwise, kWordsBool},
+    {"lookahead", &Options::lookahead, kWordsLookahead},
     {"sor_block_lb", &Options::sor_block_lb, nullptr},
     {"dist_wire_us", &Options::dist_wire_us, nullptr},
     {"dist_mirror", &Options::dist_mirror, kWordsMirror},
diff --git a/hnanosolver_amd/device.py b/hnanosolver_amd/device.py
--- a/hnanosolver_amd/device.py
+++ b/hnanosolver_amd/device.py
@@ -48,6 +48,14 @@
     outs = (C.c_void_p * max(1, n))(*[_ptr(t) for t in dsts])
     _raise(lib.hns_dev_advect_scalars(grid.ptr, _ptr(u), ins, outs, n, _ptr(sdf), int(has_collision), dt, inv_dx, current_stream()))
     return dsts
+
+
+def advect_scalars_ahead(grid: IndexGridHandle, u, srcs: Sequence, dsts: Sequence, adv_out, dt: float, inv_dx: float):
+    n = len(srcs)
+    ins = (C.c_void_p * max(1, n))(*[_ptr(t) for t in srcs])
+    outs = (C.c_void_p * max(1, n))(*[_ptr(t) for t in dsts])
+    _raise(lib.hns_dev_advect_scalars_ahead(grid.ptr, _ptr(u), ins, outs, n, _ptr(adv_out), dt, inv_dx, current_stream()))
+    return dsts, adv_out
 
 
 def divergence(grid: IndexGridHandle, u, div, inv_dx: float):
@@ -187,6 +195,14 @@
         ms, n = (C.c_float * 5)(), C.c_longlong(0)
         _raise(lib.hns_sim_stage_times(self._ptr, ms, C.byref(n)))
         return dict(zip(("advect_vector", "divergence", "pressure", "gradient", "advect_scalars"), [float(x) for x in ms])), int(n.value)
+
+    def lookahead_counts(self):
+        p, c = C.c_longlong(0), C.c_longlong(0)
+        _raise(lib.hns_sim_lookahead_counts(self._ptr, C.byref(p), C.byref(c)))
+        return int(p.value), int(c.value)
+
+    def velocity_ptr(self) -> int:
+        return int(lib.hns_sim_velocity_ptr(self._ptr) or 0)
 
     def set_active_masks(self, masks: Optional[np.ndarray], stream: int = 0) -> None:
         if masks is None:
diff --git a/include/hns.h b/include/hns.h
--- a/include/hns.h
+++ b/include/hns.h
@@ -105,6 +105,7 @@
 int hns_sim_pressure_time(hns_sim*, float* total_ms, long long* launches);
 int hns_sim_stage_timing(hns_sim*, int max_substeps);
 int hns_sim_stage_times(hns_sim*, float* ms5, long long* substeps);
+int hns_sim_lookahead_counts(hns_sim*, long long* produced, long long* consumed);
 float* hns_sim_velocity_ptr(hns_sim*);
 float* hns_sim_field_ptr(hns_sim*, const char* name);
 float* hns_sim_divergence_ptr(hns_sim*);
@@ -134,6 +135,8 @@
                           void* stream);
 int hns_dev_advect_scalars(hns_grid*, const float* vel3, const float* const* in, float* const* out, int n, const float* sdf, int has_collision,
                            float dt, float inv_dx, void* stream);
+int hns_dev_advect_scalars_ahead(hns_grid*, const float* vel3, const float* const* in, float* const* out, int n, float* adv_out3, float dt, float inv_dx,
+                                 void* stream);
 int hns_dev_divergence(hns_grid*, const float* vel3, float* div, float inv_dx, void* stream);
 int hns_dev_rbgs_color(hns_grid*, const float* div, float* p, float dx, float omega, int color, void* stream);
 int hns_dev_rbgs_iterate(hns_grid*, const float* div, float* p_a, float* p_b, float dx, float omega, int iterations, int* result_in_b,
```

Result: faster. 662.2, median of 6 (+2.3%).
